# Wumpf/yasph2d

Measured on AMD Instinct MI355X. Metric: particle-steps/sec (whole node), 2D DFSPH dam-break, higher is better.
Workload: dtype f32

## Files before the change

### include/sphx.h

```cpp
#ifndef SPHX_H
#define SPHX_H

#include <stddef.h>
#include <stdint.h>

#ifdef __cplusplus
extern "C" {
#endif

#define SPHX_ABI_VERSION 5

enum {
    SPHX_OK = 0,
    SPHX_ERR_INVALID_ARGUMENT = 1,
    SPHX_ERR_NO_DEVICE = 2,
    SPHX_ERR_HIP = 3,
    SPHX_ERR_NOT_READY = 4,
    SPHX_ERR_NONFINITE = 5,
    SPHX_ERR_NEIGHBOR_PANIC = 6,
    SPHX_ERR_CAPACITY = 7,
    SPHX_ERR_OUT_OF_DOMAIN = 8
};

enum {
// ... 91 lines not shown
typedef struct sphx_render_out {
    uint8_t* rgba;
    uint32_t* owner;
} sphx_render_out;
enum { SPHX_RENDER_NONE = 0xFFFFFFFFu, SPHX_RENDER_BOUNDARY = 0xFFFFFFFEu };
enum { SPHX_RENDER_DEVICE_POINTERS = 1u };
int sphx_render_fit(uint32_t width, uint32_t height, float x, float y, float w, float h, sphx_render_view* out);
int sphx_render(sphx_ctx* ctx, const sphx_render_view* view, uint32_t flags, const sphx_render_out* out);

typedef struct sphx_rect { float x0, y0, x1, y1; } sphx_rect;
#define SPHX_REMOVE_MAX_RECTS 8
enum { SPHX_REMOVE_OUTSIDE = 1u };
int sphx_append(sphx_ctx* ctx, const float* pos_xy, const float* vel_xy , uint32_t m, uint32_t* out_first_id );
int sphx_remove(sphx_ctx* ctx, const sphx_rect* rects, uint32_t n_rects, uint32_t flags, uint32_t* out_removed );

#define SPHX_STATE_SECTIONS 9
enum {
    SPHX_STATE_SEC_POSITIONS = 0, SPHX_STATE_SEC_VELOCITIES = 1, SPHX_STATE_SEC_PARTICLE_ID = 2, SPHX_STATE_SEC_DENSITY = 3, SPHX_STATE_SEC_ALPHA = 4,
    SPHX_STATE_SEC_KAPPA = 5, SPHX_STATE_SEC_STIFFNESS = 6, SPHX_STATE_SEC_ACCEL = 7, SPHX_STATE_SEC_BOUNDARY = 8
};
enum { SPHX_STATE_DEVICE_BUFFER = 1u };
int sphx_state_size(sphx_ctx* ctx, uint64_t* out_bytes);
int sphx_state_save(sphx_ctx* ctx, void* buf, uint64_t capacity, uint32_t flags, uint64_t* out_bytes );
int sphx_state_load(sphx_ctx* ctx, const void* buf, uint64_t bytes, uint32_t flags);
int sphx_state_digest(sphx_ctx* ctx, uint64_t* out );
int sphx_state_save_file(sphx_ctx* ctx, const char* path);
int sphx_state_load_file(sphx_ctx* ctx, const char* path);

#define SPHX_TRACK_MAX_IDS 16384
#define SPHX_TRACK_ABSENT  0xFFFFFFFFu
enum { SPHX_TRACK_DEVICE_POINTERS = 1u };
typedef struct sphx_track_out {
    uint32_t* slot;
    float* pos;
    float* vel;
    float* density;
} sphx_track_out;
typedef struct sphx_track_status { uint32_t m, recording, max_frames, every, frames, dropped, reserved[2]; } sphx_track_status;
int sphx_track_set(sphx_ctx* ctx, const uint32_t* ids , uint32_t m);
int sphx_track_fetch(sphx_ctx* ctx, uint32_t flags, const sphx_track_out* out);
int sphx_track_record(sphx_ctx* ctx, uint32_t max_frames, uint32_t every);
int sphx_track_get_status(const sphx_ctx* ctx, sphx_track_status* out);
int sphx_track_read(sphx_ctx* ctx, uint32_t first_frame, uint32_t n_frames, uint32_t flags, float* out );
int sphx_download_by_id(sphx_ctx* ctx, uint32_t first_id, uint32_t count, uint32_t flags, const sphx_track_out* out, uint32_t* out_present );

typedef struct sphx_fields_out {
    float* vel_grad;
    float* divergence;
    float* vorticity;
    float* color_grad;
} sphx_fields_out;
enum { SPHX_FIELDS_DEVICE_POINTERS = 1u };
int sphx_particle_fields(sphx_ctx* ctx, uint32_t flags, const sphx_fields_out* out);

#define SPHX_STATS_MAX_RECTS 8
enum { SPHX_STATS_DEVICE_POINTERS = 1u };
typedef struct sphx_stats_rec {
    uint64_t count;
    uint64_t nonfinite;
    uint64_t density_count;
    uint32_t density_valid;
    uint32_t reserved;
    double sum_pos[2];
    double sum_vel[2];
    double sum_speed_sq;
    double sum_angular;
    double sum_density;
    double sum_density_sq;
    double max_speed_sq;
    float min_pos[2], max_pos[2];
    float min_density, max_density;
} sphx_stats_rec;
typedef struct sphx_stats_frame { uint64_t step; float dt; uint32_t n; } sphx_stats_frame;
typedef struct sphx_stats_status { uint32_t n_rects, recording, max_frames, every, frames, dropped, reserved[2]; } sphx_stats_status;
int sphx_fluid_stats(sphx_ctx* ctx, const sphx_rect* rects , uint32_t n_rects, uint32_t flags, sphx_stats_rec* out );
int sphx_stats_record(sphx_ctx* ctx, const sphx_rect* rects , uint32_t n_rects, uint32_t max_frames, uint32_t every);
int sphx_stats_get_status(const sphx_ctx* ctx, sphx_stats_status* out);
int sphx_stats_read(sphx_ctx* ctx, uint32_t first_frame, uint32_t n_frames, sphx_stats_rec* out ,
                    sphx_stats_frame* info );

int sphx_debug_correction_counts(sphx_ctx* ctx, uint64_t out[3]);
int sphx_debug_quiet_counts(sphx_ctx* ctx, uint64_t out[2]);
int sphx_debug_takeover_counts(sphx_ctx* ctx, uint64_t out[3]);

int sphx_clear_cached(sphx_ctx* ctx);
int sphx_step_begin(sphx_ctx* ctx, float dt_prev, float* out_vmax);
int sphx_step_finish(sphx_ctx* ctx, float dt, sphx_step_stats* out_stats);

typedef struct sphx_timer_law {
    uint32_t adaptive;
    float cfl_factor;
    float particle_diameter;
    uint32_t reserved;
    uint64_t timestep_min_ns;
    uint64_t timestep_max_ns;
    uint64_t simulation_step_ns;
} sphx_timer_law;
int sphx_step_begin_law(sphx_ctx* ctx, float dt_prev, const sphx_timer_law* law, float* out_vmax);

int sphx_wcsph_step_begin(sphx_ctx* ctx, float dt, float* out_vmax);
int sphx_wcsph_step_finish(sphx_ctx* ctx, float dt, sphx_step_stats* out_stats);

int sphx_update_neighborhood(sphx_ctx* ctx);
int sphx_update_densities(sphx_ctx* ctx, int kernel_kind);
int sphx_compute_alpha(sphx_ctx* ctx);

int sphx_download_solver_state(sphx_ctx* ctx, float* alpha, float* kappa, float* stiffness);
int sphx_download_neighbors(sphx_ctx* ctx, uint16_t* counts, uint32_t* lists, uint64_t* out_total_entries);
int sphx_download_cells(sphx_ctx* ctx, int which, uint32_t* first_particle, uint32_t* cidx, uint32_t* out_count);
uint32_t sphx_last_flags(const sphx_ctx* ctx);
int sphx_grid_info(const sphx_ctx* ctx, int which, uint32_t* out4);
int sphx_get_constants(const sphx_ctx* ctx, float* out6);
int sphx_get_viscosity(const sphx_ctx* ctx, uint32_t* model, float* fluid_viscosity, float* normalizer_laplacian);


int sphx_reserve(sphx_ctx* ctx, uint32_t capacity);
int sphx_tile_configure(sphx_ctx* ctx, int axis, uint32_t cell_lo, uint32_t cell_hi, uint32_t halo_cells, int has_left, int has_right);
#define SPHX_MAX_TILE_PEERS 8
typedef struct sphx_tile_rect { uint32_t x0, x1, y0, y1; } sphx_tile_rect;
int sphx_tile_configure_rect(sphx_ctx* ctx, const sphx_tile_rect* own, uint32_t halo_cells, const sphx_tile_rect* peers, uint32_t n_peers);
int sphx_tile_pack_n(sphx_ctx* ctx, void* const* d_send, uint32_t n_send, uint32_t cap_records);
int sphx_tile_apply_n(sphx_ctx* ctx, const void* const* d_recv, uint32_t n_recv, uint32_t cap_records);
int sphx_tile_advect_pack_n(sphx_ctx* ctx, float dt, void* const* d_send, uint32_t n_send, uint32_t cap_records);
int sphx_tile_upload(sphx_ctx* ctx, const float* pos_xy, const float* vel_xy, const uint32_t* ids, uint32_t n);
#define SPHX_HALO_RECORD_BYTES 32
int sphx_tile_pack(sphx_ctx* ctx, void* d_send_left, void* d_send_right, uint32_t cap_records);
int sphx_tile_apply(sphx_ctx* ctx, const void* d_from_left, const void* d_from_right, uint32_t cap_records);
int sphx_tile_count_kept(sphx_ctx* ctx);
int sphx_sub_regrid(sphx_ctx* ctx, uint32_t* out_n_local);
int sphx_sub_regrid_div(sphx_ctx* ctx, uint32_t* out_n_local);
int sphx_sub_regrid_warm(sphx_ctx* ctx, uint32_t* out_n_local);
int sphx_sub_run_ahead(sphx_ctx* ctx, float dt_prev_of_next_step);
int sphx_tile_carry_warmstart(sphx_ctx* ctx, int kappa, int stiffness);
int sphx_tile_defer_advect(sphx_ctx* ctx, int on);
int sphx_tile_band_packs(const sphx_ctx* ctx, uint32_t* out);
int sphx_tile_send_counts(sphx_ctx* ctx, void* const* d_send, uint32_t n_send, uint32_t cap_records, uint32_t* out_counts);
int sphx_sub_nonpressure(sphx_ctx* ctx, float dt_prev, float* out_vmax_sq);
int sphx_sub_predict(sphx_ctx* ctx, float dt);
int sphx_sub_warmstart(sphx_ctx* ctx, int divergence, float dt);
int sphx_sub_iteration(sphx_ctx* ctx, int divergence, float dt, int first, double* out_err_sum, uint64_t* out_n_owned);
int sphx_sub_advect(sphx_ctx* ctx, float dt);
int sphx_sub_predict_iteration(sphx_ctx* ctx, float dt, double* out_err_sum, uint64_t* out_n_owned);


typedef struct sphx_multi sphx_multi;
enum { SPHX_LAYOUT_AUTO = 0, SPHX_LAYOUT_STRIPS = 1, SPHX_LAYOUT_GRID = 2 };
typedef struct sphx_multi_options {
    uint32_t halo_cells;
    uint32_t fixed_halo;
    uint32_t rebalance_every;
    uint32_t layout;
    uint32_t cap_records;
    uint32_t overlap_exchange;
    uint32_t reserved[2];
} sphx_multi_options;
typedef struct sphx_comm_ops {
    void* user;
    int rank, world;
    int (*exchange)(void* user, const int* peers, int n_peers, void* const* d_send, void* const* d_recv, size_t bytes, void* hip_stream);
    int (*allreduce)(void* user, const double* in, int n, int op, double* out);
    void (*abort)(void* user);
} sphx_comm_ops;
typedef struct sphx_multi_info_t {
    uint32_t world, local_tiles, halo_now, halo_max, peers, n_local, cap_records, grid_layout;
    int32_t axis;
    uint32_t band_packs;
// ... 177 lines not shown
```

### yasph2d_amd/__init__.py

```python
import ctypes as C

import numpy as np

from . import _lib
from ._lib import (FLAG_DENSITY_ITER_CAP, FLAG_DIVERGENCE_ITER_CAP, FLAG_DENSE_CELL, FLAG_NEIGHBOR_CAP, FLAG_STRAY_PARTICLES, FLAG_WARMUP, KERNEL_POLY6,
                   KERNEL_SPIKY, KERNEL_WENDLAND_C2, VISCOSITY_PHYSICAL, VISCOSITY_XSPH, SphxError, SphxKernelTime, SphxParams, SphxStepStats)

__all__ = ["SphxContext", "FluidParticleWorld", "TimeManager", "DFSPHSolver", "DFSPHMultiSolver", "default_params", "duration_from_secs_f32",
           "duration_as_secs_f32", "SphxError", "WCSPHSolver", "VISCOSITY_XSPH", "VISCOSITY_PHYSICAL", "SAMPLE_FIELDS", "gauge_elevation",
           "render_fit", "render_merge", "write_png", "SCENE_RECT", "TRACK_FIELDS", "FIELD_NAMES", "STATS_DTYPE", "STATS_FRAME_DTYPE"]


def _p(a):
    return a.ctypes.data_as(C.c_void_p) if a is not None else None


LISTS_32BIT = 0xFFFFFFFF


_VISCOSITY_MODELS = {"xsph": VISCOSITY_XSPH, "physical": VISCOSITY_PHYSICAL}


def default_params(smoothing_factor=2.0, particle_density=10000.0, fluid_density=100.0, device=0, fixed_iterations=(0, 0), viscosity="xsph",
                   fluid_viscosity=None):
# ... 440 lines not shown
            return out
        out = dict(key=np.zeros((h, w), np.uint32), owner=np.zeros((h, w), np.uint32), rgba=np.zeros((h, w, 4), np.uint8))
        o = _lib.SphxRenderLayer(*[(out[k].ctypes.data or 1) for k in ("key", "owner", "rgba")])
        self._chk(self.L.sphx_tile_render_layer(self.h, C.byref(view), 0, C.byref(o)))
        return out

    def track_record(self, max_frames, every=1):
        self._chk(self.L.sphx_track_record(self.h, max_frames, every))

    def track_frames(self, first=0, count=None):
        st = self.track_status()
        if count is None:
            count = max(st["frames"] - first, 0)
        out = np.zeros((count, st["m"], 4), np.float32)
        self._chk(self.L.sphx_track_read(self.h, first, count, 0, _p(out) if out.size else None))
        return out

    def ids_issued(self):
        first = C.c_uint32()
        rc = self.L.sphx_append(self.h, None, None, 0, C.byref(first))
        if rc == _lib.ERR_NOT_READY:
            return 0
        self._chk(rc)
        return first.value

    def download_by_id(self, first=0, count=None, fields=TRACK_FIELDS):
        if count is None:
            count = max(self.ids_issued() - first, 0)
        outs = _track_outputs(fields, count)
        present = C.c_uint32()
        self._chk(self.L.sphx_download_by_id(self.h, first, count, 0, C.byref(_track_struct(outs)), C.byref(present)))
        outs["present"] = present.value
        return outs

    def download_boundary(self):
        xy = np.zeros((self.nb, 2), np.float32)
        ids = np.zeros(self.nb, np.uint32)
        self._chk(self.L.sphx_download_boundary(self.h, _p(xy), _p(ids)))
        return xy, ids

    def download_solver_state(self):
        n = self.n
        a, k, s = (np.zeros(n, np.float32) for _ in range(3))
        self._chk(self.L.sphx_download_solver_state(self.h, _p(a), _p(k), _p(s)))
        return dict(alpha=a, kappa=k, stiffness=s)

    def download_neighbors(self):
        n = self.n
        counts = np.zeros((n, 2), np.uint16)
        total = C.c_uint64()
        self._chk(self.L.sphx_download_neighbors(self.h, _p(counts), None, C.byref(total)))
        lists = np.zeros(total.value, np.uint32)
        self._chk(self.L.sphx_download_neighbors(self.h, None, _p(lists), C.byref(total)))
        start = np.zeros(n + 1, np.uint64)
        np.cumsum(counts[:, 1].astype(np.uint64), out=start[1:])
        return counts, start, lists

    def download_cells(self, static=False):
        m = C.c_uint32()
        self._chk(self.L.sphx_download_cells(self.h, int(static), None, None, C.byref(m)))
        first = np.zeros(m.value, np.uint32)
        cidx = np.zeros(m.value, np.uint32)
        self._chk(self.L.sphx_download_cells(self.h, int(static), _p(first), _p(cidx), C.byref(m)))
        return first, cidx

    def last_flags(self):
        return self.L.sphx_last_flags(self.h)

    def correction_counts(self):
        out = (C.c_uint64 * 3)()
        self._chk(self.L.sphx_debug_correction_counts(self.h, out))
        return int(out[0]), int(out[1]), int(out[2])

    def quiet_counts(self):
        out = (C.c_uint64 * 2)()
        self._chk(self.L.sphx_debug_quiet_counts(self.h, out))
        return int(out[0]), int(out[1])

    def takeover_counts(self):
        out = (C.c_uint64 * 3)()
        self._chk(self.L.sphx_debug_takeover_counts(self.h, out))
        return int(out[0]), int(out[1]), int(out[2])

    def grid_info(self, which=0):
        out = (C.c_uint32 * 4)()
        self._chk(self.L.sphx_grid_info(self.h, which, out))
        return dict(blocks=out[0], entries=out[1], nbx=out[2], nby=out[3])

    def constants(self):
        out = np.zeros(6, np.float32)
        self._chk(self.L.sphx_get_constants(self.h, _p(out)))
        return out

    def viscosity(self):
        m, mu, nlap = C.c_uint32(), C.c_float(), C.c_float()
        self._chk(self.L.sphx_get_viscosity(self.h, C.byref(m), C.byref(mu), C.byref(nlap)))
        return {VISCOSITY_XSPH: "xsph", VISCOSITY_PHYSICAL: "physical"}[m.value], np.float32(mu.value), np.float32(nlap.value)

    def sample(self, points, kernel=KERNEL_WENDLAND_C2, fields=SAMPLE_FIELDS):
        flags = _sample_fields(fields)
        if _is_torch(points):
            import torch

            if points.device.type != "cuda" or points.dtype != torch.float32 or points.dim() != 2 or points.shape[1] != 2:
                raise ValueError("points must be a float32 [m, 2] tensor on the context's device")
            if self.params is not None and points.device.index not in (None, self.params.device):
                raise ValueError("points are on %s, the context on device %d" % (points.device, self.params.device))
            pts = points.contiguous()
            m = pts.shape[0]
            outs = _torch_outputs(flags, (m,), pts.device)
            torch.cuda.current_stream(pts.device).synchronize()
            self._chk(self.L.sphx_sample_points(self.h, C.c_void_p(pts.data_ptr()), m, kernel, _lib.SAMPLE_DEVICE_POINTERS,
                                                C.byref(_out_struct(outs, lambda t: t.data_ptr()))))
            self.synchronize()
            return outs
        pts = np.ascontiguousarray(points, np.float32)
        if pts.ndim != 2 or pts.shape[1] != 2:
            raise ValueError("points must be a float32 [m, 2] array, not shape %s" % (pts.shape,))
        m = len(pts)
        outs = _numpy_outputs(flags, (m,))
        self._chk(self.L.sphx_sample_points(self.h, _p(pts), m, kernel, 0, C.byref(_out_struct(outs, lambda a: a.ctypes.data))))
        return outs

    def sample_grid(self, origin, spacing, shape, kernel=KERNEL_WENDLAND_C2, fields=SAMPLE_FIELDS):
        flags = _sample_fields(fields)
        dx, dy = (spacing, spacing) if np.ndim(spacing) == 0 else spacing
        ny, nx = (int(v) for v in shape)
        if nx < 0 or ny < 0:
            raise ValueError("shape must be (ny, nx) with non-negative sizes")
        outs = _numpy_outputs(flags, (ny, nx))
        self._chk(self.L.sphx_sample_grid(self.h, origin[0], origin[1], dx, dy, nx, ny, kernel, 0,
                                          C.byref(_out_struct(outs, lambda a: a.ctypes.data))))
        return outs

    def render(self, view=None, *, out=None, owner=False, rgba=True, **view_fields):
        if view is None:
            width, height = view_fields.pop("width", 1920), view_fields.pop("height", 1080)
            view = render_fit(width, height, view_fields.pop("world_rect", SCENE_RECT))
        else:
            view = _copy_view(view)
        _set_view_fields(view, view_fields)
        owner_tensor = owner if _is_torch(owner) else None
        owner = owner_tensor is not None or bool(owner)
        if not rgba and not owner:
            raise ValueError("nothing to render: rgba and owner are both off")
        h, w = view.height, view.width
        o = _lib.SphxRenderOut()
        if out is not None or owner_tensor is not None:
            import torch

            dev = out.device if out is not None else owner_tensor.device
            if out is not None and (not _is_torch(out) or out.device.type != "cuda" or out.dtype != torch.uint8 or tuple(out.shape) != (h, w, 4)
                                    or not out.is_contiguous()):
                raise ValueError("out must be a contiguous uint8 (%d, %d, 4) tensor on the context's device" % (h, w))
            if not rgba and out is not None:
                raise ValueError("out given with rgba=False")
            own = None
            if owner:
                own = owner_tensor if owner_tensor is not None else torch.empty((h, w), dtype=torch.int32, device=dev)
                if own.dtype != torch.int32 or tuple(own.shape) != (h, w) or not own.is_contiguous() or own.device != dev:
                    raise ValueError("owner must be a contiguous int32 (%d, %d) tensor on the device of out" % (h, w))
            o.rgba = (out.data_ptr() or 1) if out is not None else None
            o.owner = (own.data_ptr() or 1) if own is not None else None
            torch.cuda.current_stream(dev).synchronize()
            self._chk(self.L.sphx_render(self.h, C.byref(view), _lib.RENDER_DEVICE_POINTERS, C.byref(o)))
            self.synchronize()
# ... 367 lines not shown
```

### yasph2d_amd/_lib.py

```python
import ctypes as C
import os
import subprocess

_HERE = os.path.dirname(os.path.abspath(__file__))
LIB_PATH = os.environ.get("SPHX_LIB") or os.path.join(_HERE, "libsphx.so")
CSRC = os.path.join(_HERE, "csrc")

OK, ERR_INVALID_ARGUMENT, ERR_NO_DEVICE, ERR_HIP, ERR_NOT_READY, ERR_NONFINITE, ERR_NEIGHBOR_PANIC, ERR_CAPACITY, ERR_OUT_OF_DOMAIN = range(9)
FLAG_NEIGHBOR_CAP, FLAG_DENSITY_ITER_CAP, FLAG_DIVERGENCE_ITER_CAP, FLAG_WARMUP, FLAG_STRAY_PARTICLES, FLAG_DENSE_CELL = 1, 2, 4, 8, 16, 32
KERNEL_WENDLAND_C2, KERNEL_POLY6, KERNEL_SPIKY = 0, 1, 2
VISCOSITY_XSPH, VISCOSITY_PHYSICAL = 0, 1


class SphxParams(C.Structure):
    _fields_ = [
        ("smoothing_length", C.c_float),
        ("particle_mass", C.c_float),
        ("fluid_density", C.c_float),
        ("particle_radius", C.c_float),
        ("gravity", C.c_float * 2),
        ("grid_min", C.c_float * 2),
        ("xsph_epsilon", C.c_float),
        ("max_avg_density_error", C.c_float),
        ("max_density_iterations", C.c_uint32),
# ... 137 lines not shown
    _fields_ = [("fixed", C.c_uint32), ("cfl_factor", C.c_float), ("timestep_max_ns", C.c_uint64), ("timestep_min_ns", C.c_uint64),
                ("simulation_step_ns", C.c_uint64), ("timestep_target_frame_ns", C.c_uint64), ("total_simulated_ns", C.c_uint64),
                ("num_simulation_steps", C.c_uint32), ("reserved", C.c_uint32)]


class SphxMultiOptions(C.Structure):
    _fields_ = [("halo_cells", C.c_uint32), ("fixed_halo", C.c_uint32), ("rebalance_every", C.c_uint32), ("layout", C.c_uint32),
                ("cap_records", C.c_uint32), ("overlap_exchange", C.c_uint32), ("reserved", C.c_uint32 * 2)]


COMM_EXCHANGE = C.CFUNCTYPE(C.c_int, C.c_void_p, C.POINTER(C.c_int), C.c_int, C.POINTER(C.c_void_p), C.POINTER(C.c_void_p), C.c_size_t, C.c_void_p)
COMM_ALLREDUCE = C.CFUNCTYPE(C.c_int, C.c_void_p, C.POINTER(C.c_double), C.c_int, C.c_int, C.POINTER(C.c_double))
COMM_ABORT = C.CFUNCTYPE(None, C.c_void_p)


class SphxCommOps(C.Structure):
    _fields_ = [("user", C.c_void_p), ("rank", C.c_int), ("world", C.c_int), ("exchange", COMM_EXCHANGE), ("allreduce", COMM_ALLREDUCE),
                ("abort", COMM_ABORT)]


class SphxMultiInfo(C.Structure):
    _fields_ = [("world", C.c_uint32), ("local_tiles", C.c_uint32), ("halo_now", C.c_uint32), ("halo_max", C.c_uint32), ("peers", C.c_uint32),
                ("n_local", C.c_uint32), ("cap_records", C.c_uint32), ("grid_layout", C.c_uint32), ("axis", C.c_int32), ("band_packs", C.c_uint32),
                ("exchanges", C.c_uint64), ("rebalances", C.c_uint64), ("build_particles", C.c_uint64), ("neighbor_entries", C.c_uint64),
                ("remote_entries", C.c_uint64), ("owned_local", C.c_uint64), ("transport", C.c_char * 96),
                ("halo_bytes_packed", C.c_uint64), ("halo_bytes_sent", C.c_uint64), ("ownership_seconds", C.c_double)]


LAYOUT_AUTO, LAYOUT_STRIPS, LAYOUT_GRID = 0, 1, 2

_vp, _u16p = C.c_void_p, C.c_void_p
_f, _u32, _u64, _i = C.c_float, C.c_uint32, C.c_uint64, C.c_int
class SphxTileStateOut(C.Structure):
    _fields_ = [(k, C.c_void_p) for k in ("pos", "vel", "id", "density", "alpha", "kappa", "stiffness")]


SIGNATURES = {
    "sphx_abi_version": (_u32, []),
    "sphx_default_params": (_i, [_f, _f, _f, C.POINTER(SphxParams)]),
    "sphx_create": (_i, [C.POINTER(SphxParams), C.POINTER(_vp)]),
    "sphx_destroy": (None, [_vp]),
    "sphx_last_error": (C.c_char_p, [_vp]),
    "sphx_set_boundary": (_i, [_vp, _vp, _u32]),
    "sphx_upload": (_i, [_vp, _vp, _vp, _u32]),
    "sphx_append": (_i, [_vp, _vp, _vp, _u32, C.POINTER(_u32)]),
    "sphx_remove": (_i, [_vp, C.POINTER(SphxRect), _u32, _u32, C.POINTER(_u32)]),
    "sphx_state_size": (_i, [_vp, C.POINTER(_u64)]),
    "sphx_state_save": (_i, [_vp, _vp, _u64, _u32, C.POINTER(_u64)]),
    "sphx_state_load": (_i, [_vp, _vp, _u64, _u32]),
    "sphx_state_digest": (_i, [_vp, C.POINTER(_u64)]),
    "sphx_state_save_file": (_i, [_vp, C.c_char_p]),
    "sphx_state_load_file": (_i, [_vp, C.c_char_p]),
    "sphx_track_set": (_i, [_vp, _vp, _u32]),
    "sphx_track_fetch": (_i, [_vp, _u32, C.POINTER(SphxTrackOut)]),
    "sphx_track_record": (_i, [_vp, _u32, _u32]),
    "sphx_track_get_status": (_i, [_vp, C.POINTER(SphxTrackStatus)]),
    "sphx_track_read": (_i, [_vp, _u32, _u32, _u32, _vp]),
    "sphx_particle_fields": (_i, [_vp, _u32, C.POINTER(SphxFieldsOut)]),
    "sphx_fluid_stats": (_i, [_vp, C.POINTER(SphxRect), _u32, _u32, _vp]),
    "sphx_stats_record": (_i, [_vp, C.POINTER(SphxRect), _u32, _u32, _u32]),
    "sphx_stats_get_status": (_i, [_vp, C.POINTER(SphxStatsStatus)]),
    "sphx_stats_read": (_i, [_vp, _u32, _u32, _vp, _vp]),
    "sphx_tile_fluid_stats": (_i, [_vp, C.POINTER(SphxRect), _u32, _u32, _vp]),
    "sphx_tile_stats_record": (_i, [_vp, C.POINTER(SphxRect), _u32, _u32, _u32]),
    "sphx_tile_stats_frame": (_i, [_vp, _f, _u32]),
    "sphx_tile_stats_read": (_i, [_vp, _u32, _u32, _vp, _vp]),
    "sphx_multi_fluid_stats": (_i, [_vp, C.POINTER(SphxRect), _u32, _u32, _vp, _vp]),
    "sphx_multi_stats_record": (_i, [_vp, C.POINTER(SphxRect), _u32, _u32, _u32]),
    "sphx_multi_stats_get_status": (_i, [_vp, C.POINTER(SphxStatsStatus)]),
    "sphx_multi_stats_read": (_i, [_vp, _u32, _u32, _vp, _vp]),
    "sphx_tile_state_pack": (_i, [_vp, _u32, C.POINTER(SphxTileStateOut), C.POINTER(_u64), C.POINTER(_u32)]),
    "sphx_tile_state_fetch": (_i, [_vp, C.POINTER(_u64), C.POINTER(_u32)]),
    "sphx_tile_upload_state": (_i, [_vp, _vp, _vp, _vp, _vp, _vp, _u32]),
    "sphx_get_tiling_invariant": (_i, [_vp]),
    "sphx_multi_state_size": (_i, [_vp, C.POINTER(_u64)]),
    "sphx_multi_state_save": (_i, [_vp, _vp, _u64, _u32, C.POINTER(_u64)]),
    "sphx_multi_state_load": (_i, [_vp, C.POINTER(_vp), C.POINTER(_u64), _u32, _u32]),
    "sphx_multi_state_digest": (_i, [_vp, C.POINTER(_u64)]),
    "sphx_multi_state_save_file": (_i, [_vp, C.c_char_p]),
    "sphx_multi_state_load_file": (_i, [_vp, C.c_char_p]),
    "sphx_debug_correction_counts": (_i, [_vp, _vp]),
    "sphx_debug_quiet_counts": (_i, [_vp, _vp]),
    "sphx_debug_takeover_counts": (_i, [_vp, _vp]),
    "sphx_download_by_id": (_i, [_vp, _u32, _u32, _u32, C.POINTER(SphxTrackOut), C.POINTER(_u32)]),
    "sphx_download": (_i, [_vp, _vp, _vp, _vp, _vp]),
    "sphx_download_boundary": (_i, [_vp, _vp, _vp]),
    "sphx_num_particles": (_u32, [_vp]),
    "sphx_num_boundary": (_u32, [_vp]),
    "sphx_sample_points": (_i, [_vp, _vp, _u32, _i, _u32, C.POINTER(SphxSampleOut)]),
    "sphx_sample_grid": (_i, [_vp, _f, _f, _f, _f, _u32, _u32, _i, _u32, C.POINTER(SphxSampleOut)]),
    "sphx_render_fit": (_i, [_u32, _u32, _f, _f, _f, _f, C.POINTER(SphxRenderView)]),
    "sphx_render": (_i, [_vp, C.POINTER(SphxRenderView), _u32, C.POINTER(SphxRenderOut)]),
    "sphx_multi_render": (_i, [_vp, C.POINTER(SphxRenderView), _u32, C.POINTER(SphxRenderOut)]),
    "sphx_multi_render_layer": (_i, [_vp, C.POINTER(SphxRenderView), _u32, C.POINTER(SphxRenderLayer)]),
    "sphx_render_merge": (_i, [_u32, _u32, C.POINTER(SphxRenderLayer), _u32, C.POINTER(SphxRenderLayer)]),
    "sphx_tile_render_layer": (_i, [_vp, C.POINTER(SphxRenderView), _u32, C.POINTER(SphxRenderLayer)]),
    "sphx_tile_render_window": (_i, [_vp, C.POINTER(SphxRenderView), _u32, C.POINTER(_u32), C.POINTER(SphxRenderLayer)]),
    "sphx_clear_cached": (_i, [_vp]),
    "sphx_step_begin": (_i, [_vp, _f, C.POINTER(_f)]),
    "sphx_step_begin_law": (_i, [_vp, _f, _vp, _vp]),
    "sphx_timer_law_of": (_i, [_vp, _f, _vp]),
    "sphx_timer_set_target_frame": (None, [_vp, _u64]),
    "sphx_timer_on_step_started": (None, [_vp]),
    "sphx_step_finish": (_i, [_vp, _f, C.POINTER(SphxStepStats)]),
    "sphx_update_neighborhood": (_i, [_vp]),
    "sphx_update_densities": (_i, [_vp, _i]),
    "sphx_compute_alpha": (_i, [_vp]),
    "sphx_download_solver_state": (_i, [_vp, _vp, _vp, _vp]),
    "sphx_download_neighbors": (_i, [_vp, _vp, _vp, C.POINTER(_u64)]),
    "sphx_download_cells": (_i, [_vp, _i, _vp, _vp, C.POINTER(_u32)]),
    "sphx_grid_info": (_i, [_vp, _i, C.POINTER(_u32)]),
    "sphx_last_flags": (_u32, [_vp]),
    "sphx_get_constants": (_i, [_vp, _vp]),
    "sphx_get_viscosity": (_i, [_vp, C.POINTER(_u32), C.POINTER(_f), C.POINTER(_f)]),
    "sphx_reserve": (_i, [_vp, _u32]),
    "sphx_tile_configure": (_i, [_vp, _i, _u32, _u32, _u32, _i, _i]),
    "sphx_tile_upload": (_i, [_vp, _vp, _vp, _vp, _u32]),
    "sphx_tile_pack": (_i, [_vp, _vp, _vp, _u32]),
    "sphx_tile_apply": (_i, [_vp, _vp, _vp, _u32]),
    "sphx_tile_count_kept": (_i, [_vp]),
    "sphx_sub_regrid": (_i, [_vp, C.POINTER(_u32)]),
    "sphx_sub_regrid_div": (_i, [_vp, C.POINTER(_u32)]),
    "sphx_sub_regrid_warm": (_i, [_vp, C.POINTER(_u32)]),
    "sphx_sub_nonpressure": (_i, [_vp, _f, C.POINTER(_f)]),
    "sphx_sub_predict": (_i, [_vp, _f]),
    "sphx_sub_warmstart": (_i, [_vp, _i, _f]),
    "sphx_sub_iteration": (_i, [_vp, _i, _f, _i, C.POINTER(C.c_double), C.POINTER(_u64)]),
    "sphx_sub_predict_iteration": (_i, [_vp, _f, C.POINTER(C.c_double), C.POINTER(_u64)]),
    "sphx_tile_band_packs": (_i, [_vp, C.POINTER(_u32)]),
    "sphx_tile_send_counts": (_i, [_vp, _vp, _u32, _u32, C.POINTER(_u32)]),
    "sphx_sub_advect": (_i, [_vp, _f]),
    "sphx_shm_open": (_vp, [C.c_char_p, _i, _i]),
    "sphx_shm_allreduce": (_i, [_vp, _vp, _i, _i, _vp]),
    "sphx_shm_allgather": (_i, [_vp, _vp, _i, _vp]),
    "sphx_shm_abort": (None, [_vp]),
    "sphx_sub_run_ahead": (_i, [_vp, C.c_float]),
    "sphx_tile_carry_warmstart": (_i, [_vp, _i, _i]),
    "sphx_set_tiling_invariant": (_i, [_vp, _i]),
    "sphx_tile_defer_advect": (_i, [_vp, _i]),
    "sphx_build_stats": (_i, [_vp, _vp, _vp, _vp]),
    "sphx_shm_close": (None, [_vp]),
    "sphx_tile_configure_rect": (_i, [_vp, _vp, _u32, _vp, _u32]),
    "sphx_tile_pack_n": (_i, [_vp, _vp, _u32, _u32]),
    "sphx_tile_apply_n": (_i, [_vp, _vp, _u32, _u32]),
    "sphx_tile_advect_pack_n": (_i, [_vp, _f, _vp, _u32, _u32]),
    "sphx_view_request": (_i, [_vp, _u32, C.POINTER(_u32)]),
    "sphx_view_fetch": (_i, [_vp, _i, C.POINTER(C.POINTER(_f)), C.POINTER(_u32)]),
    "sphx_synchronize": (_i, [_vp]),
    "sphx_set_stream": (_i, [_vp, _vp]),
    "sphx_profile_enable": (_i, [_vp, _i]),
    "sphx_profile_reset": (_i, [_vp]),
    "sphx_profile_filter": (_i, [_vp, C.c_char_p, _u32]),
    "sphx_profile_get": (_i, [_vp, _vp, C.POINTER(_u32)]),
    "sphx_profile_event_overhead": (_i, [_vp, C.POINTER(C.c_double)]),
    "sphx_multi_default_options": (_i, [C.POINTER(SphxMultiOptions)]),
    "sphx_multi_create": (_i, [C.POINTER(SphxParams), C.POINTER(C.c_int), _i, C.POINTER(SphxMultiOptions), C.POINTER(_vp)]),
    "sphx_multi_create_rank": (_i, [C.POINTER(SphxParams), _i, C.POINTER(SphxCommOps), C.c_char_p, _i, _i, C.POINTER(SphxMultiOptions), C.POINTER(_vp)]),
    "sphx_multi_destroy": (None, [_vp]),
    "sphx_multi_last_error": (C.c_char_p, [_vp]),
    "sphx_multi_set_layout": (_i, [_vp, _i, _vp, _u32]),
    "sphx_multi_set_grid_layout": (_i, [_vp, _u32, _u32, _vp, _vp]),
    "sphx_multi_set_boundary": (_i, [_vp, _vp, _u32]),
    "sphx_multi_upload": (_i, [_vp, _vp, _vp, _vp, _u32]),
    "sphx_multi_clear_cached": (_i, [_vp]),
    "sphx_multi_step_begin": (_i, [_vp, _f, C.POINTER(_f)]),
    "sphx_multi_step_finish": (_i, [_vp, _f, C.POINTER(SphxStepStats)]),
# ... 87 lines not shown
```

### yasph2d_amd/csrc/sphx_handoff.hpp

```cpp
#pragma once
#include <cstdint>
#include <cstring>

namespace sphx {

struct BuildHandoff {
    enum Kind : uint8_t { None, WarmApplied, FirstErrors };
    Kind kind = None;
    bool has_flags = false, warm_taken = false;
    uint32_t mark_tag = 0;
    struct Taken {
        bool fused, flags_usable, warm_taken;
    };
    static BuildHandoff warm_applied() { return BuildHandoff{WarmApplied, false, false, 0u}; }
    static BuildHandoff first_errors(bool flags, uint32_t tag, bool taken) { return BuildHandoff{FirstErrors, flags, flags && taken, tag}; }
    void clear() { *this = BuildHandoff{}; }
    bool first_errors_pending() const { return kind == FirstErrors; }
    bool take_warm() {
        const bool applied = kind == WarmApplied;
        if (applied) clear();
        return applied;
    }
    Taken take_first_errors(bool first_divergence, uint32_t rseq) {
        if (kind != FirstErrors || !first_divergence) return Taken{false, false, false};
        const bool usable = has_flags && mark_tag == rseq;
        const Taken t{true, usable, usable && warm_taken};
        clear();
        return t;
    }
};

class PendingCount {
  public:
    enum class Maker : uint8_t { Nobody, Correction, Pack, Classifier };
    PendingCount() = default;
    void made_by_correction(uint32_t n) { *this = PendingCount(Maker::Correction, n); }
    void made_by_pack(uint32_t n) { *this = PendingCount(Maker::Pack, n); }
    void made_by_classifier(uint32_t n, float dt) { *this = PendingCount(Maker::Classifier, n, true, bits(dt)); }
    bool live() const { return maker_ != Maker::Nobody; }
    bool from_classifier() const { return maker_ == Maker::Classifier; }
    bool is_for(uint32_t n) const { return live() && n_ == n; }
    bool is_for_first_of(uint32_t n) const { return live() && n_ <= n; }
    uint32_t n() const { return n_; }
    bool take_over_class(uint32_t n, float dt) {
        const bool mine = from_classifier() && takeable_ && n_ == n && dt_bits_ == bits(dt);
        if (mine) made_by_pack(n);
        return mine;
    }
    void bar_take_over() { takeable_ = false; }
    bool drop() {
        const bool wipe = live();
        forget();
        return wipe;
    }
    bool drop_if_from_classifier() { return from_classifier() && drop(); }
    void forget() { *this = PendingCount(); }

  private:
    PendingCount(Maker m, uint32_t n, bool takeable = false, uint32_t dt_bits = 0) : maker_(m), takeable_(takeable), n_(n), dt_bits_(dt_bits) {}
    static uint32_t bits(float f) {
        uint32_t u;
        std::memcpy(&u, &f, 4);
        return u;
    }
    Maker maker_ = Maker::Nobody;
    bool takeable_ = false;
    uint32_t n_ = 0, dt_bits_ = 0;
};

}
```

### yasph2d_amd/csrc/sphx_internal.hpp

```cpp
#pragma once
#include <hip/hip_runtime.h>

#include <dlfcn.h>

#include <algorithm>
#include <cstdint>
#include <cstdlib>
#include <cstdio>
#include <cstring>
#include <functional>
#include <map>
#include <string>
#include <vector>

#include "../../include/sphx.h"
#include "sphx_handoff.hpp"

namespace sphx {

constexpr uint32_t EMPTY = 0xFFFFFFFFu;
constexpr uint32_t MAX_NEIGHBORS = 64;
constexpr uint32_t BLOCK_SHIFT = 6;
constexpr uint32_t BLOCK_CELLS = 4096;
constexpr uint32_t SCAN_TILE = 4096;
// ... 27 lines not shown
constexpr uint32_t RANK_LOOP_MAX = 4096;
constexpr uint32_t LOOP_HIST = 512;

constexpr uint32_t MAX_TILE_PEERS = 8;
struct TileRect {
    uint32_t x0, x1, y0, y1;
};

struct Consts {
    float h;
    float radius_sq;
    float cell_inv;
    float gmin_x, gmin_y;
    float w_hinv, w_norm, w_ngrad;
    float p6_hsq, p6_norm, p6_ngrad;
    float sp_h, sp_norm, sp_ngrad;
    float mass, rho0, xsph_eps;
    float ax, ay;
    float gx, gy;
    float wc_stiffness, wc_boundary_force;
    TileRect tile;
    uint32_t remote_cap;
    uint32_t q_noclamp;
    uint32_t nt_cold;
    uint32_t xcd_shift;
    uint32_t rev;
};

struct ViscConsts {
    uint32_t visc_model;
    float mu;
    float vis_nlap;
};
template <int VM>
struct ViscArg {};
template <>
struct ViscArg<SPHX_VISCOSITY_PHYSICAL> : ViscConsts {};

struct NbView {
    const uint32_t* list;
    const uint16_t* counts;
    const uint32_t* wave;
    const uint32_t* remote;
    uint32_t lazy_hi;
    uint32_t stream;
};
constexpr uint32_t COUNT_MANY_LINES = 1u << 14;
struct PVr {
    const float2* pos;
    const float2* vel;
};

struct GridView {
    const uint32_t* dir;
    const uint2* fine;
    uint32_t bx0, by0, nbx, nby;
    uint32_t cbits;
};
struct NbGrid {
    const uint32_t* dirn;
    const uint2* fine;
    uint32_t bx0, by0, nbx, nbx1, nby1;
};
constexpr uint32_t DIRN_FLAG = 1u;

struct alignas(128) Stripe {
    unsigned long long nb_entries;
    unsigned long long owned;
    unsigned long long rem_entries;
    unsigned long long res_hi, res_lo;
    uint32_t ticket;
    uint32_t pad0;
    unsigned long long zs_skipped, zs_window, zs_remote;
    unsigned long long zs_quiet;
    uint32_t pad[12];
};
static_assert(sizeof(Stripe) == 128, "one stripe, one cache line");
struct alignas(128) VmaxStripe {
    uint32_t vmax[4];
    uint32_t pad[28];
};
struct alignas(128) MarkStripe {
    uint32_t knz_mark;
    uint32_t pad[31];
};
struct alignas(128) SpecLine {
    uint32_t flags;
    uint32_t pad0;
    unsigned long long moved;
    uint32_t pad[28];
};
struct DevScalars {
    uint32_t flags;
    uint32_t ticket;
    uint32_t sort_total;
    float dt;
    uint32_t loop_done;
    uint32_t pad0;
    unsigned long long snap_hi[2], snap_lo[2];
    uint32_t pad[18];
    Stripe stripe[STRIPES];
    VmaxStripe vstripe[STRIPES];
    MarkStripe mstripe[STRIPES];
    SpecLine spec;
};

struct Mailbox {
    volatile uint32_t seq;
    uint32_t flags;
    uint32_t vmax_sq_bits;
    uint32_t quiet_seq;
    double err_sum;
    unsigned long long nb_entries;
    unsigned long long owned_cum;
    unsigned long long rem_entries;
    uint32_t sort_total;
    uint32_t dt_bits;
    unsigned long long dt_ns;
    volatile uint32_t loop_gen_done;
    uint32_t loop_iters;
    double loop_hist[LOOP_HIST];
    uint32_t send_counts[MAX_TILE_PEERS];
};

struct ResArgs {
    uint32_t enabled;
    uint32_t rseq;
    Mailbox* mb;
    uint32_t seq;
};
struct VmaxArgs {
    uint32_t enabled;
    uint32_t vslot;
    Mailbox* mb;
    uint32_t seq;
};
struct LoopArgs {
    uint32_t enabled;
    uint32_t iter;
    uint32_t fixed;
    uint32_t max_iters;
    uint32_t gen;
    uint32_t n_total;
    float tol;
    float rho0;
    float dt;
};

struct TimerLaw {
    uint32_t enabled, adaptive;
    float cfl_factor, particle_diameter;
    unsigned long long min_ns, max_ns, step_ns;
};

struct Grid {
    uint32_t* dir = nullptr;
    uint32_t* dirn = nullptr;
    uint32_t dir_cap = 0;
    uint2* fine = nullptr;
    uint32_t* hist = nullptr;
    uint32_t* tile_empty = nullptr;
    uint32_t tile_cap = 0;
    uint32_t fine_cap = 0;
    uint32_t bx0 = 0, by0 = 0, nbx = 0, nby = 0, nblk = 0;
    std::vector<uint8_t> cover;
    std::vector<uint32_t> h_dir;
    bool fine_valid = false;
    uint32_t len() const { return nblk * BLOCK_CELLS; }
    uint32_t cbits_floor = 1;
    uint32_t cbits() const {
        uint32_t b = cbits_floor < 1u ? 1u : cbits_floor > 31u ? 31u : cbits_floor;
        while (b < 31u && ((1u << b) - 1u) < len()) ++b;
        return b;
    }
    GridView view() const { return GridView{dir, fine, bx0, by0, nbx, nby, cbits()}; }
    NbGrid nview() const { return nbx && nby ? NbGrid{dirn, fine, bx0, by0, nbx, nbx - 1u, nby - 1u} : NbGrid{dirn, fine, 0u, 0u, 1u, 0u, 0u}; }
};

struct ProfTotals {
    uint64_t launches = 0;
    double ms = 0, bytes = 0;
};
struct ProfPending {
    const char* name;
    double bytes;
    hipEvent_t a, b;
};

}

struct sphx_ctx {
    sphx_params P;
    sphx::Consts K;
    sphx::ViscConsts VK;
    int device = 0;
    hipStream_t stream = nullptr;
    std::string err;

    uint32_t N = 0, capN = 0;
    uint32_t B = 0, capB = 0;
    uint32_t cached_n = 0;
    bool set_changed = false;
    uint64_t ids_issued = 0;
    uint32_t* edit_buf = nullptr;
    uint32_t edit_cap = 0;
    struct Track {
        uint32_t m = 0, unique = 0, log2_bits = 0;
        uint32_t* set_buf = nullptr;
        uint32_t *table = nullptr, *map = nullptr, *filter = nullptr, *found = nullptr;
        float* rec = nullptr;
        uint32_t recording = 0, max_frames = 0, every = 0, frames = 0, dropped = 0, steps = 0;
        uint32_t* scratch = nullptr;
        size_t scratch_cap = 0;
    } track;
    struct Stats {
        sphx_stats_rec* scratch = nullptr;
        sphx_stats_rec* rec = nullptr;
        sphx_rect rects[SPHX_STATS_MAX_RECTS] = {};
        uint32_t n_rects = 0, recording = 0, max_frames = 0, every = 0, frames = 0, dropped = 0, steps = 0;
        std::vector<sphx_stats_frame> info;
    } stats;
    bool uploaded = false, boundary_changed = true, tails_dirty = true, in_step = false;
    bool lists_current = false;
    unsigned long long* state_dig = nullptr;
    uint32_t* mstate_buf = nullptr;
    size_t mstate_cap = 0;
    uint32_t mstate_n = 0;
    uint32_t fast_walk_ok = 0;
    uint32_t sample_ready = 0;
    bool tile_density_ready = false;
    const char* sample_missing = "no neighbour build yet: run a step, or sphx_update_neighborhood + sphx_update_densities";
    float* sample_buf = nullptr;
    size_t sample_cap = 0;
    uint32_t* render_buf = nullptr;
    size_t render_cap = 0;
    float* fields_buf = nullptr;
    size_t fields_cap = 0;
    uint32_t num_density_iters = 1, num_divergence_iters = 0;
    float step_dt_prev = 0, step_vmax = 0;
    uint32_t step_flags = 0;

    float2 *posA = nullptr, *posA2 = nullptr;
    float2 *vel = nullptr, *vel2 = nullptr;
    sphx::PVr pv() const { return sphx::PVr{posA, vel}; }
    float* kbuf = nullptr;
    uint32_t* knz = nullptr;
    int zero_skip = -1;
    bool zero_skip_on() const { return zero_skip < 0 ? N >= 4000000u : zero_skip != 0; }
    int zero_skip_count = 0;
    bool quiet_hint[2] = {false, false};
    unsigned long long qf_launches = 0;
    int quiet_takeover = 1;
    uint32_t thin_grid = 0;
    int quiet_takeover_density = 1;
    bool take_over(bool divergence) const {
        return !tile_mode && (divergence || quiet_takeover_density) && (quiet_takeover == 2 || (quiet_takeover == 1 && quiet_hint[divergence ? 1 : 0]));
    }
    unsigned long long thin_launches = 0, takeover_producers = 0;
    float2* accel = nullptr;
    float *density = nullptr, *alpha = nullptr, *alpha2 = nullptr, *kappa = nullptr, *stiff = nullptr;
    float *kappa2 = nullptr, *stiff2 = nullptr;
    uint32_t *pid = nullptr, *pid2 = nullptr;
    uint32_t *key = nullptr, *slot = nullptr, *order = nullptr;
    uint32_t idx_cap = 0;
    uint32_t soff() const { return capN; }
    float2 *bpos = nullptr, *bpos2 = nullptr;
    uint32_t *bid = nullptr, *bid2 = nullptr;
    sphx::Grid gdyn, gstat;
    bool have_fluid_bbox = false;
    uint32_t fb[4] = {0, 0, 0, 0};
    uint32_t builds_since_cover = 0;
    bool need_expand = false;
    bool need_recover = false;
    uint32_t recover_streak = 0;
    uint32_t recover_cooldown = 0;
    std::vector<float> h_boundary;
    uint32_t* nb_list = nullptr;
    uint16_t* nb_counts = nullptr;
    uint32_t* nb_wave = nullptr;
    uint32_t* nb_remote = nullptr;
    uint32_t pre_seq = 0, pre_warm = 0, law_dt_bits = 0;
    bool law_active = false;
    uint32_t pre_gen = 0;
    uint32_t pre_queued = 0;
    uint32_t loop_gen = 0;
    uint32_t res_seq = 0;
    uint32_t vmax_seq = 0;
    struct RunAhead {
        bool queued = false;
        bool valid = false;
        uint32_t n = 0, dt_bits = 0, vslot = 0;
        uint32_t seq = 0;
    } ahead;
    float tile_pending_dt = 0.0f;
    uint32_t tile_pending_n = 0;
    bool tile_defer_advect = false;
    float sub_ahead_dt = 0.0f;
    bool tile_carry_kappa = true, tile_carry_stiff = true;
    bool tiling_invariant = false;
    int run_ahead = 1;
#ifndef SPHX_DEFAULT_FUSE_PREDICT
#define SPHX_DEFAULT_FUSE_PREDICT 1
#endif
    int fuse_predict = SPHX_DEFAULT_FUSE_PREDICT;
    int tile_fuse_class = 1;
    uint32_t tile_band_packs = 0;
    bool tile_fix_owner = false;
    int fuse_div = 1;
    int xcd_chunk = -1;
    int alternate_sweep = 1;
    int fuse_warm = 1;
    sphx::BuildHandoff handoff;
    int host_loop = 0;
    std::string prof_filter;
    uint32_t prof_every = 1, prof_counter = 0;
    bool external_stream = false;
    hipStream_t view_stream = nullptr;
    hipEvent_t view_packed = nullptr, view_done = nullptr;
    float *view_dev = nullptr, *view_host = nullptr;
    uint32_t view_cap = 0, view_count = 0;
    bool view_pending = false;
    uint32_t wcsph_n = 0;
    bool in_wcsph = false;
    int lazy_table = 1;
    int stream_lists = -1;
    int nt_cold_stores = -1;
    sphx::NbView nbv() const {
        return sphx::NbView{nb_list, nb_counts, nb_wave, nb_remote, (uint32_t)lazy_table, stream_lists < 0 ? (N >= 4000000u ? 1u : 0u) : (uint32_t)stream_lists};
    }
    uint32_t* scan_partials = nullptr;
    uint32_t scan_partials_cap = 0;
    unsigned long long* scan_state = nullptr;
    uint32_t scan_state_cap = 0, scan_epoch = 0;
    sphx::PendingCount pending;
    int no_fused_count = 0;
    int scan_two_pass = 0;
    sphx::DevScalars* d_scal = nullptr;
    sphx::Mailbox* mbox = nullptr;
    sphx::Mailbox* mbox_dev = nullptr;
    uint32_t seq = 0;
    unsigned long long nb_cum = 0, nb_last = 0;
    unsigned long long rem_cum = 0, rem_last = 0;
    unsigned long long owned_cum = 0, owned_last = 0, owned_base = 0;
    bool owned_dirty = false;
    bool tile_mode = false;
    uint32_t tile_halo = 0;
    uint32_t tile_npeers = 0;
    sphx::TileRect tile_peer[sphx::MAX_TILE_PEERS] = {};
    uint32_t n_owned = 0;
    uint32_t* tile_blk = nullptr;
    bool tile_strip_left = false, tile_strip_right = false;

    bool profiling = false;
    std::vector<hipEvent_t> ev_pool;
    std::vector<sphx::ProfPending> prof_pending;
    std::map<std::string, sphx::ProfTotals> prof_totals;

    int fail(int code, const char* what, const char* detail = nullptr) {
        quiet_hint[0] = quiet_hint[1] = false;
        err = what;
        if (detail) {
            err += ": ";
            err += detail;
        }
        return code;
    }
};
```

### yasph2d_amd/csrc/sphx_kernels.hip

```cpp
#include "sphx_internal.hpp"
#include "sphx_sqrt.hpp"
#include "sphx_xcd.hpp"

namespace sphx {

__device__ __forceinline__ uint32_t part1by1(uint32_t x) {
    x &= 0xffffu;
    x = (x ^ (x << 8)) & 0x00ff00ffu;
    x = (x ^ (x << 4)) & 0x0f0f0f0fu;
    x = (x ^ (x << 2)) & 0x33333333u;
    x = (x ^ (x << 1)) & 0x55555555u;
    return x;
}
__device__ __forceinline__ uint32_t morton2(uint32_t x, uint32_t y) { return (part1by1(y) << 1) | part1by1(x); }

__device__ __forceinline__ uint32_t spread6(uint32_t v) {
    v &= 63u;
    v = (v | (v << 4)) & 0x30Fu;
    v = (v | (v << 2)) & 0x333u;
    v = (v | (v << 1)) & 0x555u;
    return v;
}
__device__ __forceinline__ uint32_t sat_u16(float v) {
    v = fminf(fmaxf(v, 0.0f), 65535.0f);
// ... 558 lines not shown
    }
    count_cell(K, g, i < n, i, p, hist, cidx, slot, ring, scal);
}

constexpr uint32_t ORDER_HEAD = 0x80000000u, ORDER_INDEX = 0x7FFFFFFFu;
#ifndef SPHX_SCATTER_PER_LANE
#define SPHX_SCATTER_PER_LANE 4
#endif
constexpr uint32_t SCATTER_PER_LANE = SPHX_SCATTER_PER_LANE;
__global__ __launch_bounds__(256) void k_scatter(const uint32_t* __restrict__ cidx, const uint32_t* __restrict__ slot, uint32_t n,
                                                  const uint2* __restrict__ fine, uint32_t* __restrict__ order, uint32_t cbits,
                                                  uint32_t* __restrict__ hist, uint32_t rev) {
    const uint32_t b0 = xcd_bid(xcd_packed_rev(rev), xcd_packed_shift(rev)) * (256u * SCATTER_PER_LANE) + threadIdx.x;
    if (b0 - threadIdx.x >= n) return;
    uint32_t w[SCATTER_PER_LANE];
#pragma unroll
    for (uint32_t u = 0; u < SCATTER_PER_LANE; ++u) w[u] = b0 + u * 256u < n ? cidx[b0 + u * 256u] : EMPTY;
    uint32_t first[SCATTER_PER_LANE];
#pragma unroll
    for (uint32_t u = 0; u < SCATTER_PER_LANE; ++u) first[u] = fine[w[u] == EMPTY ? 0u : w[u] & ((1u << cbits) - 1u)].x;
#ifdef SPHX_SLOT_AT_COUNT
    (void)hist;
#pragma unroll
    for (uint32_t u = 0; u < SCATTER_PER_LANE; ++u) {
        if (w[u] == EMPTY) continue;
        const uint32_t i = b0 + u * 256u;
        uint32_t sl = w[u] >> cbits;
        if (sl == cell_slot_max(cbits)) sl = slot[i];
        const uint32_t p = first[u] + sl;
        if (p < n) order[p] = i | (sl == 0u ? ORDER_HEAD : 0u);
    }
#else
    (void)slot;
    const uint32_t lane = threadIdx.x & 63u;
    uint32_t old[SCATTER_PER_LANE], pos_in_run[SCATTER_PER_LANE];
#pragma unroll
    for (uint32_t u = 0; u < SCATTER_PER_LANE; ++u) {
        const uint32_t idx = w[u];
        const uint32_t prev = dpp_mov<0x138>(idx, idx);
        const bool head = (lane == 0) || (idx != prev);
        const unsigned long long mask = __ballot(head);
        const uint32_t start = 63u - (uint32_t)__clzll(mask & (~0ull >> (63u - lane)));
        const unsigned long long rest = (lane == 63) ? 0ull : (mask >> (lane + 1));
        const uint32_t end = rest ? lane + (uint32_t)__ffsll((long long)rest) : 64u;
        uint32_t o = 0;
        if (head && idx != EMPTY) o = atomicSub(&hist[idx], end - lane);
        old[u] = o;
        pos_in_run[u] = (start << 8) | (lane - start);
    }
#pragma unroll
    for (uint32_t u = 0; u < SCATTER_PER_LANE; ++u) {
        const uint32_t o = (uint32_t)__shfl((int)old[u], (int)(pos_in_run[u] >> 8), 64);
        if (w[u] == EMPTY) continue;
        const uint32_t i = b0 + u * 256u;
        const uint32_t sl = o - 1u - (pos_in_run[u] & 0xFFu);
        const uint32_t p = first[u] + sl;
        if (p < n) order[p] = i | (sl == 0u ? ORDER_HEAD : 0u);
    }
#endif
}

struct GatherArgs {
    const float2* pos_in;
    float2* pos_out;
    const float2* vel_in;
    float2* vel_out;
    const float* r_in;
    float* r_out;
    const float* r2_in;
    float* r2_out;
    const float* r3_in;
    float* r3_out;
    const uint32_t* u_in;
    uint32_t* u_out;
    DevScalars* count_owned;
    DevScalars* flags;
    float advect_dt;
    uint32_t advect_below;
    uint32_t fix_owner;
    float cell_inv, gmin_x, gmin_y;
    TileRect own;
    uint32_t rank_by_id;
    uint32_t nt_cold;
};
#ifndef SPHX_GATHER_PER_LANE
#define SPHX_GATHER_PER_LANE 1
#endif
constexpr uint32_t GATHER_PER_LANE = SPHX_GATHER_PER_LANE;
__global__ __launch_bounds__(256) void k_rank_gather(const uint32_t* __restrict__ order, const uint32_t* __restrict__ cidx, uint32_t n,
                                                      uint32_t n_in, const uint2* __restrict__ fine, GatherArgs a,
                                                      const uint32_t* __restrict__ n_dev, uint32_t cbits, uint32_t rev) {
    if (n_dev) n = min(n, *n_dev);
    const uint32_t b0 = xcd_bid(xcd_packed_rev(rev), xcd_packed_shift(rev)) * (256u * GATHER_PER_LANE);
    if (b0 >= n) return;
    constexpr int RANK_L = 5, RANK_R = 6;
    constexpr uint32_t ORD_HALO = 8, SPAN = 256u * GATHER_PER_LANE;
    static_assert(RANK_L <= (int)ORD_HALO && RANK_R <= (int)ORD_HALO, "window of order[] words in LDS");
    __shared__ uint32_t sord[SPAN + 2 * ORD_HALO];
    uint32_t own[GATHER_PER_LANE];
#pragma unroll
    for (uint32_t u = 0; u < GATHER_PER_LANE; ++u) {
        own[u] = order[min(b0 + u * 256u + threadIdx.x, n - 1u)];
        sord[ORD_HALO + u * 256u + threadIdx.x] = own[u];
    }
    if (threadIdx.x < 2 * ORD_HALO) {
        const int32_t k = threadIdx.x < ORD_HALO ? (int32_t)(b0 + threadIdx.x) - (int32_t)ORD_HALO : (int32_t)(b0 + SPAN + threadIdx.x - ORD_HALO);
        sord[threadIdx.x < ORD_HALO ? threadIdx.x : SPAN + threadIdx.x] = order[(uint32_t)min(max(k, 0), (int32_t)n - 1)];
    }
    bool ok[GATHER_PER_LANE];
    float2 q[GATHER_PER_LANE], v[GATHER_PER_LANE];
    float r1[GATHER_PER_LANE], r2[GATHER_PER_LANE], r3[GATHER_PER_LANE];
    uint32_t id[GATHER_PER_LANE];
#pragma unroll
    for (uint32_t u = 0; u < GATHER_PER_LANE; ++u) {
        const uint32_t i = own[u] & ORDER_INDEX;
        ok[u] = b0 + u * 256u + threadIdx.x < n && i < n_in;
        const uint32_t ic = ok[u] ? i : 0u;
        q[u] = a.pos_in[ic];
        v[u] = a.vel_in ? a.vel_in[ic] : make_float2(0.0f, 0.0f);
        r1[u] = a.r_in ? a.r_in[ic] : 0.0f, r2[u] = a.r2_in ? a.r2_in[ic] : 0.0f, r3[u] = a.r3_in ? a.r3_in[ic] : 0.0f;
        id[u] = a.u_in ? a.u_in[ic] : 0u;
    }
    __syncthreads();
#pragma unroll
    for (uint32_t u = 0; u < GATHER_PER_LANE; ++u) {
        if (!ok[u]) continue;
        const uint32_t p = b0 + u * 256u + threadIdx.x, i = own[u] & ORDER_INDEX;
        uint32_t near[RANK_L + RANK_R + 1];
#pragma unroll
        for (int d = -RANK_L; d <= RANK_R; ++d) near[d + RANK_L] = sord[(int)(ORD_HALO + u * 256u + threadIdx.x) + d];
        uint32_t heads_l = 0, heads_r = 0;
#pragma unroll
        for (int d = 0; d <= RANK_L; ++d) heads_l |= (near[RANK_L - d] >> 31) << d;
#pragma unroll
        for (int d = 1; d <= RANK_R; ++d) heads_r |= ((near[RANK_L + d] >> 31) | (p + (uint32_t)d >= n ? 1u : 0u)) << (d - 1);
        uint32_t dst;
        if (heads_l != 0u && heads_r != 0u && !(a.rank_by_id && a.u_in)) {
            const uint32_t below = (uint32_t)__builtin_ctz(heads_l), above = (uint32_t)__builtin_ctz(heads_r) + 1u;
            uint32_t rank = 0;
#pragma unroll
            for (int d = -RANK_L; d <= RANK_R; ++d) {
                if (d == 0) continue;
                const bool mate = d < 0 ? (uint32_t)(-d) <= below : (uint32_t)d < above;
                rank += (mate && (near[d + RANK_L] & ORDER_INDEX) < i) ? 1u : 0u;
            }
            dst = p - below + rank;
        } else {
            const uint32_t cw = cidx[i];
            if (cw == EMPTY) continue;
            const uint2 se = fine[cw & ((1u << cbits) - 1u)];
            const uint32_t s = se.x;
            uint32_t e = se.y;
            if (e > n) e = n;
            if (e - s <= RANK_LOOP_MAX && a.rank_by_id && a.u_in) {
                const uint32_t me = id[u] & 0x7FFFFFFFu;
                uint32_t rank = 0;
                for (uint32_t k = s; k < e; ++k) {
                    const uint32_t j = order[k] & ORDER_INDEX;
                    const uint32_t idj = j < n_in ? a.u_in[j] & 0x7FFFFFFFu : 0xFFFFFFFFu;
                    rank += (j != i && (idj < me || (idj == me && j < i))) ? 1u : 0u;
                }
                dst = s + rank;
            } else if (e - s <= RANK_LOOP_MAX) {
                uint32_t rank = 0;
#pragma unroll
                for (int d = -RANK_L; d <= RANK_R; ++d) {
                    const int32_t k = (int32_t)p + d;
                    rank += (k >= (int32_t)s && k < (int32_t)e && (near[d + RANK_L] & ORDER_INDEX) < i) ? 1u : 0u;
                }
                for (uint32_t k = s; k + RANK_L < p && k < e; ++k) rank += ((order[k] & ORDER_INDEX) < i) ? 1u : 0u;
                for (uint32_t k = max(s, p + RANK_R + 1u); k < e; ++k) rank += ((order[k] & ORDER_INDEX) < i) ? 1u : 0u;
                dst = s + rank;
            } else {
                dst = p;
                if ((__hip_atomic_load(&a.flags->flags, __ATOMIC_RELAXED, __HIP_MEMORY_SCOPE_AGENT) & DF_DENSE_CELL) == 0u) atomicOr(&a.flags->flags, DF_DENSE_CELL);
            }
        }
        if (dst >= n) continue;
        float2 qd = q[u];
        if (a.vel_in) {
            if (a.advect_dt > 0.0f && i < a.advect_below) {
                qd.x = qd.x + v[u].x * a.advect_dt;
                qd.y = qd.y + v[u].y * a.advect_dt;
            }
            a.vel_out[dst] = v[u];
        }
        a.pos_out[dst] = qd;
        if (a.r_in) a.r_out[dst] = r1[u];
        if (a.r2_in) a.r2_out[dst] = r2[u];
        if (a.r3_in) a.r3_out[dst] = r3[u];
        if (a.u_in) {
            uint32_t idd = id[u];
            if (a.fix_owner && i < a.advect_below) {
                const uint32_t cx = sat_u16((qd.x - a.gmin_x) * a.cell_inv), cy = sat_u16((qd.y - a.gmin_y) * a.cell_inv);
                if (!rect_has(a.own, cx, cy, 0u)) idd &= 0x7FFFFFFFu;
            }
            store_cold(&a.u_out[dst], idd, a.nt_cold);
            if (a.count_owned) {
                const unsigned long long m = __ballot((idd >> 31) != 0);
                if (m && (threadIdx.x & 63) == (uint32_t)(__ffsll((long long)__ballot(1)) - 1))
                    atomicAdd(&a.count_owned->stripe[blockIdx.x % STRIPES].owned, (unsigned long long)__popcll(m));
            }
        }
    }
}

__global__ __launch_bounds__(256) void k_iota(uint32_t* __restrict__ a, uint32_t n) {
    const uint32_t i = blockIdx.x * 256 + threadIdx.x;
    if (i < n) a[i] = i;
}
__global__ __launch_bounds__(256) void k_fill_f32(float* __restrict__ a, uint32_t from, uint32_t n, float v) {
    const uint32_t i = from + blockIdx.x * 256 + threadIdx.x;
    if (i < n) a[i] = v;
}
__global__ __launch_bounds__(256) void k_advect(float2* __restrict__ posA, const float2* __restrict__ vel, uint32_t n, float dt) {
    const uint32_t i = xcd_bid() * 256 + threadIdx.x;
    if (i >= n) return;
    float2 p = posA[i];
    const float2 v = vel[i];
    p.x = p.x + v.x * dt;
    p.y = p.y + v.y * dt;
    posA[i] = p;
}
struct HaloRec {
    float4 pv;
    uint32_t id;
    float kappa, stiff;
    uint32_t pad;
};
struct TilePeers {
    uint32_t n;
    TileRect rect[MAX_TILE_PEERS];
    HaloRec* out[MAX_TILE_PEERS];
};
__device__ __forceinline__ uint32_t tile_send_mask(const Consts& K, const TileRect* rect, uint32_t nrect, uint32_t halo, float4 pv, uint32_t id) {
    const bool owned = (id >> 31) != 0 && pv.x == pv.x;
    if (!owned) return 0u;
    uint32_t cx, cy;
    cell_of(K, make_float2(pv.x, pv.y), cx, cy);
    uint32_t m = 0;
    for (uint32_t k = 0; k < nrect; ++k) m |= rect_has(rect[k], cx, cy, halo) ? (1u << k) : 0u;
    return m;
}
__device__ __forceinline__ uint32_t tile_send_mask(const Consts& K, const TilePeers& P, uint32_t halo, float4 pv, uint32_t id) {
    return tile_send_mask(K, P.rect, P.n, halo, pv, id);
}
struct TileClassArgs {
    const uint32_t* pid;
    uint32_t* blk;
    uint32_t* any;
    uint32_t halo, n;
    TileRect rect[MAX_TILE_PEERS];
};
__device__ __forceinline__ float4 tile_advected(float4 pv, float dt) {
    if (dt > 0.0f) {
        pv.x = pv.x + pv.z * dt;
        pv.y = pv.y + pv.w * dt;
    }
    return pv;
}
__global__ __launch_bounds__(256) void k_tile_count(PVr PV, const uint32_t* __restrict__ pid, uint32_t n, Consts K,
                                                     uint32_t halo, TilePeers P, uint32_t* __restrict__ blk, float dt) {
    __shared__ uint32_t wc[4][MAX_TILE_PEERS];
    const uint32_t i = blockIdx.x * 256 + threadIdx.x;
    const uint32_t m = i < n ? tile_send_mask(K, P, halo, tile_advected(ldpv(PV, i), dt), pid[i]) : 0u;
    for (uint32_t k = 0; k < P.n; ++k) {
        const uint32_t c = (uint32_t)__popcll(__ballot((m >> k) & 1u));
        if ((threadIdx.x & 63) == 0) wc[threadIdx.x >> 6][k] = c;
    }
    __syncthreads();
    if (threadIdx.x < P.n) blk[(size_t)blockIdx.x * MAX_TILE_PEERS + threadIdx.x] = wc[0][threadIdx.x] + wc[1][threadIdx.x] + wc[2][threadIdx.x] + wc[3][threadIdx.x];
}
__global__ __launch_bounds__(1024) void k_tile_offsets(uint32_t* __restrict__ blk, uint32_t nb, TilePeers P) {
    __shared__ uint32_t part[1024];
    const uint32_t per = (nb + 1023u) / 1024u;
    const uint32_t b0 = threadIdx.x * per, b1 = min(b0 + per, nb);
    for (uint32_t k = 0; k < P.n; ++k) {
        uint32_t acc = 0;
        for (uint32_t b = b0; b < b1; ++b) acc += blk[(size_t)b * MAX_TILE_PEERS + k];
        part[threadIdx.x] = acc;
        __syncthreads();
        for (uint32_t off = 1; off < 1024; off <<= 1) {
            const uint32_t v = threadIdx.x >= off ? part[threadIdx.x - off] : 0u;
            __syncthreads();
            part[threadIdx.x] += v;
            __syncthreads();
// ... 1125 lines not shown
}
__device__ __forceinline__ uint32_t wave_vmax_get(const DevScalars* __restrict__ scal, uint32_t vslot) {
    const uint32_t lane = threadIdx.x & 63u;
    const uint32_t b = lane < STRIPES ? scal->vstripe[lane].vmax[vslot & 3u] : 0u;
    return wave_max_u32(b);
}
__device__ __forceinline__ void vmax_publish(DevScalars* __restrict__ scal, const VmaxArgs& va, uint32_t bits, const TimerLaw& law, unsigned long long ns,
                                             float dt_new) {
    if (threadIdx.x < STRIPES) __hip_atomic_store(&scal->vstripe[threadIdx.x].vmax[(va.vslot + 2u) & 3u], 0u, __ATOMIC_RELAXED, __HIP_MEMORY_SCOPE_AGENT);
    if (threadIdx.x == 0) {
        va.mb->vmax_sq_bits = bits;
        if (law.enabled) {
            __hip_atomic_store((uint32_t*)&scal->dt, __float_as_uint(dt_new), __ATOMIC_RELAXED, __HIP_MEMORY_SCOPE_AGENT);
            va.mb->dt_ns = ns;
            va.mb->dt_bits = __float_as_uint(dt_new);
        }
    }
    publish_common(scal, va.mb, va.seq);
}

__device__ __forceinline__ unsigned long long residual_fixed(float e, bool& bad) {
    bad = !(e < 1073741824.0f);
    const float t = __builtin_rintf((bad ? 0.0f : e) * 16777216.0f);
    const uint32_t bits = __float_as_uint(t);
    const uint32_t m = (bits & 0x7fffffu) | 0x800000u;
    const int sh = (int)((bits >> 23) & 0xffu) - 150;
    unsigned long long f = sh >= 0 ? (unsigned long long)m << (sh & 63) : (unsigned long long)(m >> min(-sh, 31));
    return (bits & 0x7f800000u) ? f : 0ull;
}
__device__ __forceinline__ void block_residual_add(float e, DevScalars* __restrict__ scal) {
    bool bad;
    const unsigned long long f = wave_sum_u63(residual_fixed(e, bad));
    __shared__ unsigned long long ws[4];
    if ((threadIdx.x & 63) == 0) ws[threadIdx.x >> 6] = f;
    if (__any(bad) && (threadIdx.x & 63) == 0) atomicOr(&scal->flags, DF_NONFINITE);
    __syncthreads();
    if (threadIdx.x == 0) {
        const unsigned long long t = ws[0] + ws[1] + ws[2] + ws[3];
        Stripe* st = &scal->stripe[blockIdx.x % STRIPES];
        if (t >> 32) atomicAdd(&st->res_hi, t >> 32);
        if (t & 0xffffffffull) atomicAdd(&st->res_lo, t & 0xffffffffull);
    }
}
__device__ __forceinline__ void residual_stripe_load(const DevScalars* __restrict__ scal, unsigned long long& hi, unsigned long long& lo) {
    const uint32_t lane = threadIdx.x & 63u;
    hi = lane < STRIPES ? scal->stripe[lane].res_hi : 0ull;
    lo = lane < STRIPES ? scal->stripe[lane].res_lo : 0ull;
}
__device__ __forceinline__ void residual_wave_reduce(unsigned long long& hi, unsigned long long& lo) {
    hi = wave_sum_u63(hi);
    lo = wave_sum_u63(lo);
}
__device__ __forceinline__ double residual_sum_f64(unsigned long long hi, unsigned long long lo, unsigned long long hi0, unsigned long long lo0) {
    return ((double)(hi - hi0) * 4294967296.0 + (double)(lo - lo0)) * (1.0 / 16777216.0);
}

__global__ __launch_bounds__(256) void k_block_occupancy(const uint2* __restrict__ fine, uint32_t nblk, uint8_t* __restrict__ occ) {
    const uint32_t b = blockIdx.x * 256 + threadIdx.x;
    if (b >= nblk) return;
    occ[b] = fine[(size_t)b * BLOCK_CELLS].x != fine[(size_t)b * BLOCK_CELLS + BLOCK_CELLS - 1].y ? 1 : 0;
}

__global__ __launch_bounds__(64) void k_clear_vmax_slot(DevScalars* scal, uint32_t vslot) {
    if (threadIdx.x < STRIPES) __hip_atomic_store(&scal->vstripe[threadIdx.x].vmax[vslot & 3u], 0u, __ATOMIC_RELAXED, __HIP_MEMORY_SCOPE_AGENT);
}

__global__ __launch_bounds__(64) void k_publish_vmax(DevScalars* scal, VmaxArgs va) {
    const uint32_t b = wave_vmax_get(scal, va.vslot);
    vmax_publish(scal, va, b, TimerLaw{}, 0ull, 0.0f);
}

#ifndef NONP_BOUNDS
#define NONP_BOUNDS __launch_bounds__(256) __attribute__((amdgpu_waves_per_eu(8, 8)))
#endif
__device__ __forceinline__ float physical_visc(const Consts& K, const ViscConsts& V, float mu_m, float r, float rho_j) {
    return mu_m * (V.vis_nlap * (K.h - r)) / rho_j;
}
template <int VM>
__global__ NONP_BOUNDS void k_nonpressure(PVr PV, const float* __restrict__ density, uint32_t n, uint32_t soff, Consts K,
                                                      float dt, NbView nb, float2* __restrict__ accel, DevScalars* __restrict__ scal, uint32_t vslot,
                                                      ViscArg<VM> V) {
    __shared__ Stage<2, 1> rec;
    const uint32_t blk = xcd_bid(K.rev, K.xcd_shift);
    const uint32_t i = blk * 256 + threadIdx.x;
    NbHead h = nb_head(nb, blk, i, n);
    struct StageRec {
        float4 pv;
        float rho;
    };
    nb_stage(
        h, nb, blk, i, n, [&](uint32_t g) { return StageRec{ldpv(PV, g), gat(density, g < soff ? g : 0u)}; },
        [&](uint32_t g) {
            const Pair<float4> pv = ldpv2(PV, g);
            const Pair<float> rho = gat2(density, g < soff ? g : 0u);
            return Pair<StageRec>{StageRec{pv.a, rho.a}, StageRec{pv.b, rho.b}};
        },
        [&](uint32_t slot, const StageRec& r) {
            rec.put_vec01(slot, r.pv);
            rec.put_scal<0>(slot, r.rho);
        });
    __syncthreads();
    float vsq = 0.0f;
    if (i < n) {
        const uint32_t oi = (i - h.lw0) * 4u;
        const float4 pvi = h.wide ? ldpv(PV, i) : rec.vec01(oi);
        const uint32_t cd = h.cd;
        float ax = K.ax, ay = K.ay;
        struct Rec {
            float4 pv;
            float rho;
        };
        if constexpr (VM == SPHX_VISCOSITY_PHYSICAL) {
            const float mu_m = V.mu * K.mass;
            auto walk = [&](auto fast) {
                auto consume = [&](const Rec& r, uint32_t) {
                    const float dx = r.pv.x - pvi.x, dy = r.pv.y - pvi.y;
                    const float r_sq = dx * dx + dy * dy;
                    const float f = physical_visc(K, V, mu_m, sqrt_dist<decltype(fast)::value>(r_sq), r.rho);
                    ax = ax + f * (r.pv.z - pvi.z);
                    ay = ay + f * (r.pv.w - pvi.w);
                };
                nb_traverse(
                    h, cd, [&](uint32_t o) { return Rec{rec.vec01(o), rec.scal<0>(o)}; },
                    [&](uint32_t g) { return Rec{ldpv(PV, g), gat(density, g)}; }, consume);
            };
            if (K.q_noclamp)
                walk(std::true_type{});
            else
                walk(std::false_type{});
        } else {
            const float em = K.xsph_eps * K.mass;
            auto consume = [&](const Rec& r, uint32_t) {
                const float dx = r.pv.x - pvi.x, dy = r.pv.y - pvi.y;
                const float r_sq = dx * dx + dy * dy;
                const float f = em * poly6_eval(K, r_sq) / (r.rho * dt);
                ax = ax + f * (r.pv.z - pvi.z);
                ay = ay + f * (r.pv.w - pvi.w);
            };
            nb_traverse(
                h, cd, [&](uint32_t o) { return Rec{rec.vec01(o), rec.scal<0>(o)}; },
                [&](uint32_t g) { return Rec{ldpv(PV, g), gat(density, g)}; }, consume);
        }
        accel[i] = make_float2(ax, ay);
        const float px = pvi.z + ax * dt, py = pvi.w + ay * dt;
        vsq = tile_owns(K, pvi.x, pvi.y) ? px * px + py * py : 0.0f;
    }
    block_vmax_add(vsq, scal, vslot, (uint32_t*)&rec.raw[0]);
}

__global__ __launch_bounds__(256) void k_predict(float2* __restrict__ vel, const float2* __restrict__ accel, uint32_t n, float dt,
                                                  DevScalars* __restrict__ scal, VmaxArgs va, TimerLaw law) {
    const uint32_t i = xcd_bid() * 256 + threadIdx.x;
    const uint32_t il = min(i, n - 1u);
    float2 v = vel[il];
    const float2 a = accel[il];
    if (va.enabled) {
        __shared__ float dt_s;
        if (threadIdx.x < 64) {
            const uint32_t b = wave_vmax_get(scal, va.vslot);
            unsigned long long ns = 0;
            float d = dt;
            if (law.enabled) {
                ns = timer_law_step_ns(law, sqrtf(__uint_as_float(b)));
                d = duration_as_secs_f32(ns);
            }
            if (threadIdx.x == 0) dt_s = d;
            if (blockIdx.x == 0) vmax_publish(scal, va, b, law, ns, d);
        }
        __syncthreads();
        dt = dt_s;
    }
    if (i >= n) return;
    v.x = v.x + a.x * dt;
    v.y = v.y + a.y * dt;
    vel[i] = v;
}

__global__ __launch_bounds__(256) void k_wcsph_leapfrog1(float2* __restrict__ vel, float2* __restrict__ posA, const float2* __restrict__ accel,
                                                          uint32_t n, float dt) {
    const uint32_t i = xcd_bid() * 256 + threadIdx.x;
    if (i >= n) return;
    const float2 p0 = posA[i], v0 = vel[i];
    float4 pv = make_float4(p0.x, p0.y, v0.x, v0.y);
    const float2 a = accel[i];
    const float hdt = 0.5f * dt;
    pv.z = pv.z + hdt * a.x;
    pv.w = pv.w + hdt * a.y;
    pv.x = pv.x + pv.z * dt;
    pv.y = pv.y + pv.w * dt;
    vel[i] = make_float2(pv.z, pv.w);
    posA[i] = make_float2(pv.x, pv.y);
}
__device__ __forceinline__ float powi7(float a) {
    float r = a;
    a = a * a;
    r = r * a;
    a = a * a;
    return r * a;
}
__device__ __forceinline__ float wcsph_pressure(const Consts& K, float local_density) {
    return K.wc_stiffness * (powi7(fmaxf(local_density / K.rho0, 1.0f)) - 1.0f);
}
template <int VM>
__global__ TRAV_BOUNDS void k_wcsph_accel(PVr PV, const float* __restrict__ density, uint32_t n, uint32_t soff, Consts K,
                                          float dt, NbView nb, float2* __restrict__ accel, DevScalars* __restrict__ scal, uint32_t vslot,
                                          ViscArg<VM> V) {
    __shared__ Stage<2, 1> rec;
    const uint32_t blk = xcd_bid(K.rev, K.xcd_shift);
    const uint32_t i = blk * 256 + threadIdx.x;
    NbHead h = nb_head(nb, blk, i, n);
    struct StageRec {
        float4 pv;
        float rho;
    };
    nb_stage(
        h, nb, blk, i, n, [&](uint32_t g) { return StageRec{ldpv(PV, g), gat(density, g < soff ? g : 0u)}; },
        [&](uint32_t g) {
            const Pair<float4> pv = ldpv2(PV, g);
            const Pair<float> rho = gat2(density, g < soff ? g : 0u);
            return Pair<StageRec>{StageRec{pv.a, rho.a}, StageRec{pv.b, rho.b}};
        },
        [&](uint32_t slot, const StageRec& r) {
            rec.put_vec01(slot, r.pv);
            rec.put_scal<0>(slot, r.rho);
        });
    __syncthreads();
    float vsq = 0.0f;
    if (i < n) {
        const uint32_t oi = (i - h.lw0) * 4u;
        const float4 pvi = h.wide ? ldpv(PV, i) : rec.vec01(oi);
// ... 288 lines not shown
```

### yasph2d_amd/csrc/sphx_launch.inc

```
#include <algorithm>
#include <cmath>

using namespace sphx;

static std::string g_create_error;

#define SPHX_HIP(ctx, expr)                                                        \
    do {                                                                           \
        hipError_t e__ = (expr);                                                   \
        if (e__ != hipSuccess) return (ctx)->fail(SPHX_ERR_HIP, #expr, hipGetErrorString(e__)); \
    } while (0)

namespace {

inline uint32_t nblocks(uint32_t n, uint32_t per = 256) {
    const uint32_t b = (n + per - 1) / per;
    return per == 256 ? (b + 7u) & ~7u : b;
}
inline double kbar_of(const sphx_ctx* c) { return (c->N && c->nb_last) ? (double)c->nb_last / (double)c->N : 12.0; }
inline double list_bytes(const sphx_ctx* c) {
    if (!c->K.remote_cap) return 2.0 + 4.0 * kbar_of(c);
    const double rbar = c->N ? (double)c->rem_last / (double)c->N : 0.5;
    return 2.0 + 4.0 / 64.0 + (4.0 / 3.0) * kbar_of(c) + 4.0 * rbar + 4.0 / 256.0;
}
// ... 413 lines not shown
    if (!got) {
        SPHX_HIP(c, hipStreamSynchronize(c->stream));
        if (!reached()) return c->fail(SPHX_ERR_HIP, "device did not publish the step scalars (kernel fault?)");
    }
    __atomic_thread_fence(__ATOMIC_ACQUIRE);
    const unsigned long long cum = c->mbox->nb_entries;
    if (cum != c->nb_cum) {
        c->nb_last = cum - c->nb_cum;
        c->nb_cum = cum;
    }
    const unsigned long long rm = c->mbox->rem_entries;
    if (rm != c->rem_cum) {
        c->rem_last = rm - c->rem_cum;
        c->rem_cum = rm;
    }
    const unsigned long long ow = c->mbox->owned_cum;
    if (ow != c->owned_cum) {
        c->owned_last = ow - c->owned_cum;
        c->owned_cum = ow;
    }
    const uint32_t f = c->mbox->flags;
    if (f) hipLaunchKernelGGL(k_clear_flags, dim3(1), dim3(1), 0, c->stream, c->d_scal, f);
    if (f & DF_NB_CAP) c->step_flags |= SPHX_FLAG_NEIGHBOR_CAP;
    if (f & DF_HALO_CAP) return c->fail(SPHX_ERR_CAPACITY, "halo exchange buffer too small for the particles near a tile cut");
    if (f & DF_NEAR_EDGE) c->need_expand = true;
    if (f & DF_STRAY) {
        c->step_flags |= SPHX_FLAG_STRAY_PARTICLES;
        c->need_recover = true;
    }
    if (f & DF_DENSE_CELL) c->step_flags |= SPHX_FLAG_DENSE_CELL;
    if (f & DF_SCAN_STALL) return c->fail(SPHX_ERR_HIP, "the cell-table scan stalled waiting for a predecessor workgroup");
    if (f & DF_NONFINITE) return c->fail(SPHX_ERR_NONFINITE, "a solver residual is not finite (dfsph.rs:223 / :378 assert)");
    if (f & DF_OUT_OF_DOMAIN) return c->fail(SPHX_ERR_OUT_OF_DOMAIN, "a particle left the Morton domain the grid tables were sized for, or has no cell at all (a NaN position)");
    if (f & DF_NB_PANIC) return c->fail(SPHX_ERR_NEIGHBOR_PANIC, "64 dynamic neighbours and a static hit (neighborhood_search.rs:373 panics here)");
    return SPHX_OK;
}

int publish_and_wait(sphx_ctx* c) {
    const uint32_t seq = ++c->seq;
    hipLaunchKernelGGL(k_publish, dim3(1), dim3(64), 0, c->stream, c->d_scal, c->mbox_dev, seq);
    return wait_mailbox(c, seq);
}

void wipe_histogram(sphx_ctx* c, Grid& g) {
    if (g.hist && g.len()) hipMemsetAsync(g.hist, 0, (size_t)g.len() * 4, c->stream);
}
void drop_fused_count(sphx_ctx* c) {
    if (c->pending.drop()) wipe_histogram(c, c->gdyn);
}
void clear_histograms(sphx_ctx* c) {
    c->pending.forget();
    for (Grid* g : {&c->gdyn, &c->gstat}) wipe_histogram(c, *g);
}

void drop_class_count(sphx_ctx* c) {
    if (c->pending.drop_if_from_classifier()) wipe_histogram(c, c->gdyn);
}
void flush_pending_advect(sphx_ctx* c) {
    if (c->pending.from_classifier() || c->tile_pending_dt > 0.0f) (void)hipSetDevice(c->device);
    drop_class_count(c);
    if (!(c->tile_pending_dt > 0.0f)) return;
    const uint32_t n = c->tile_pending_n;
    const float dt = c->tile_pending_dt;
    c->tile_pending_dt = 0.0f;
    c->tile_pending_n = 0;
    const bool fix = c->tile_fix_owner;
    c->tile_fix_owner = false;
    if (!n) return;
    if (fix) {
        TilePeers none{};
        hipLaunchKernelGGL(k_tile_pack, dim3(nblocks(n)), dim3(256), 0, c->stream, (const float2*)c->vel, c->posA, c->pid, (const float*)c->kappa,
                           (const float*)c->stiff, n, c->K, c->tile_halo, none, (const uint32_t*)c->tile_blk, 0u, dt, CountArgs{}, c->d_scal, 1u,
                           (const uint32_t*)nullptr);
        return;
    }
    hipLaunchKernelGGL(k_advect, dim3(nblocks(n)), dim3(256), 0, c->stream, c->posA, (const float2*)c->vel, n, dt);
}

void sub_step_enter(sphx_ctx* c) {
    c->ahead.valid = false;
    flush_pending_advect(c);
}

int build_grid(sphx_ctx* c, Grid& g, const float2* pos, uint32_t n, const GatherArgs& ga, float advect_dt, bool ring, uint32_t* tile_n = nullptr) {
    hipStream_t st = c->stream;
    DevScalars* ds = c->d_scal;
    const uint32_t len = g.len();
    const uint32_t nt = nblocks(len, c->scan_two_pass ? SCAN_TILE : SCAN1_TILE);
    const bool counted = &g == &c->gdyn && advect_dt > 0 && !tile_n && c->pending.is_for(n);
    const bool partial = &g == &c->gdyn && tile_n && advect_dt == 0.0f && !counted && c->pending.is_for_first_of(n);
    const uint32_t first = partial ? c->pending.n() : 0u;
    if (counted || partial)
        c->pending.forget();
    else
        drop_fused_count(c);
    if (n > first && !counted) {
        const uint32_t gbc = std::max(1u, nblocks(n - first));
        if (advect_dt > 0)
            launch(c, "advect+cell_count", (16.0 + 4 + 4) * n, [&] {
                hipLaunchKernelGGL(k_key_count<true>, dim3(gbc), dim3(256), 0, st, c->pv(), (const float2*)nullptr, n, advect_dt, c->K,
                                   g.view(), g.hist, c->key, c->slot, ring ? 1u : 0u, ds, first);
            });
        else
            launch(c, "cell_count", (8.0 + 4 + 4) * (n - first), [&] {
                hipLaunchKernelGGL(k_key_count<false>, dim3(gbc), dim3(256), 0, st, PVr{nullptr, nullptr}, pos, n, 0.0f, c->K, g.view(),
                                   g.hist, c->key, c->slot, ring ? 1u : 0u, ds, first);
            });
    }
    if (!len) hipMemsetAsync(&ds->sort_total, 0, 4, st);
    uint32_t scan_seq = 0;
    if (len)
        launch(c, "cell_scan", (c->scan_two_pass ? 20.0 : 16.0) * len, [&] {
            if (c->scan_two_pass) {
                hipLaunchKernelGGL(k_scan_reduce, dim3(nt), dim3(256), 0, st, (const uint32_t*)g.hist, len, c->scan_partials, ds, &ds->sort_total);
                hipLaunchKernelGGL(k_scan_apply, dim3(nt), dim3(256), 0, st, g.hist, g.fine, len, (const uint32_t*)c->scan_partials);
                hipMemsetAsync(g.tile_empty, 0, (size_t)g.tile_cap * 4, st);
            } else {
                if (++c->scan_epoch == 0) c->scan_epoch = 1;
                if (tile_n) scan_seq = ++c->seq;
                hipLaunchKernelGGL(k_scan_onepass, dim3(nt), dim3(256), 0, st, g.hist, g.fine, len, c->scan_state, c->scan_epoch, ds, &ds->sort_total,
                                   tile_n ? c->mbox_dev : (Mailbox*)nullptr, scan_seq, g.tile_empty, tile_n ? 0xFFFFFFFFu : n);
            }
        });
    g.fine_valid = len != 0;
    if (n) {
        launch(c, "cell_scatter", 12.0 * n, [&] {
            hipLaunchKernelGGL(k_scatter, dim3((nblocks(n, 256 * SCATTER_PER_LANE) + 7u) & ~7u), dim3(256), 0, st, (const uint32_t*)c->key, (const uint32_t*)c->slot, n, (const uint2*)g.fine,
                               c->order, g.cbits(), g.hist, xcd_scatter_pack(c->K.rev, xcd_shift_of(c)));
        });
        const uint32_t ng = n;
        if (tile_n) {
            if (scan_seq) {
                *tile_n = scan_seq;
            } else {
                const uint32_t seq = ++c->seq;
                hipLaunchKernelGGL(k_publish, dim3(1), dim3(64), 0, st, ds, c->mbox_dev, seq);
                *tile_n = seq;
            }
        }
        const uint32_t gb2 = std::max(8u, (nblocks(ng, 256 * GATHER_PER_LANE) + 7u) & ~7u);
        double gbytes = 4;
        gbytes += ga.vel_in ? (16 + 16) : 16;
        if (ga.r_in) gbytes += 8;
        if (ga.r2_in) gbytes += 8;
        if (ga.r3_in) gbytes += 8;
        if (ga.u_in) gbytes += 8;
        if (ng)
            launch(c, "gather_attributes", gbytes * ng, [&] {
                hipLaunchKernelGGL(k_rank_gather, dim3(gb2), dim3(256), 0, st, (const uint32_t*)c->order, (const uint32_t*)c->key, ng, n,
                                   (const uint2*)g.fine, ga, tile_n ? (const uint32_t*)&ds->sort_total : (const uint32_t*)nullptr, g.cbits(), xcd_pack(c->K.rev, xcd_shift_of(c)));
            });
    }
    return SPHX_OK;
}

int ensure_index_scratch(sphx_ctx* c) {
    const uint32_t need = std::max(std::max(std::max(c->N, c->capN), c->B), 1u);
    if (need <= c->idx_cap) return SPHX_OK;
    int rc;
    if ((rc = dev_alloc(c, &c->key, need))) return rc;
#ifdef SPHX_SLOT_AT_COUNT
    if ((rc = dev_alloc(c, &c->slot, need))) return rc;
#endif
    if ((rc = dev_alloc(c, &c->order, need))) return rc;
    SPHX_HIP(c, hipMemsetAsync(c->order, 0, (size_t)need * 4, c->stream));
    c->idx_cap = need;
    return SPHX_OK;
}

static inline void sample_went_stale(sphx_ctx* c, const char* missing) {
    c->sample_ready = 0u;
    c->tile_density_ready = false;
    c->sample_missing = missing;
}
static inline void sample_after_step(sphx_ctx* c) {
    if (c->sample_ready == 1u)
        c->sample_ready = 2u;
    else
        sample_went_stale(c, "no neighbour build has run since the particles or the boundary changed (a step over zero fluid particles runs "
                             "none): call sphx_update_neighborhood + sphx_update_densities");
}
void track_take_frame(sphx_ctx* c);
static inline void track_after_step(sphx_ctx* c) {
    if (c->track.recording) track_take_frame(c);
}
void stats_take_frame(sphx_ctx* c, float dt);
static inline void stats_after_step(sphx_ctx* c, float dt) {
    if (c->stats.recording) stats_take_frame(c, dt);
}
static inline void lists_went_stale(sphx_ctx* c) {
    c->K.q_noclamp = 0u;
    c->lists_current = false;
    c->quiet_hint[0] = c->quiet_hint[1] = false;
    if (c->d_scal) hipMemsetAsync(&c->d_scal->spec.flags, 0, sizeof(uint32_t), c->stream);
    if (c->sample_ready) sample_went_stale(c, "the positions changed since the last neighbour build: run a step, or sphx_update_neighborhood + sphx_update_densities");
}

int ensure_nb_arrays(sphx_ctx* c, uint32_t needN, uint32_t needB, bool keep_fluid) {
    const uint32_t newN = std::max(c->capN, needN), newB = std::max(c->capB, std::max(needB, 1u));
    if (newN == c->capN && newB == c->capB && c->vel) return SPHX_OK;
    const size_t tot = (size_t)newN + newB;
    if (tot >= ((size_t)1 << 28)) return c->fail(SPHX_ERR_CAPACITY, "more than 2^28 fluid + boundary slots in one context: split the domain into tiles");
    float2* old_pos = c->posA;
    float2* old_vel = c->vel;
    c->posA = nullptr;
    c->vel = nullptr;
    int rc;
    if ((rc = dev_alloc(c, &c->posA, tot + 4)) || (rc = dev_alloc(c, &c->posA2, tot + 4)) || (rc = dev_alloc(c, &c->vel, tot)) ||
        (rc = dev_alloc(c, &c->vel2, tot)))
        return rc;
    if (keep_fluid && c->N && old_vel) {
        SPHX_HIP(c, hipMemcpyAsync(c->posA, old_pos, (size_t)c->N * 8, hipMemcpyDeviceToDevice, c->stream));
        SPHX_HIP(c, hipMemcpyAsync(c->vel, old_vel, (size_t)c->N * 8, hipMemcpyDeviceToDevice, c->stream));
        SPHX_HIP(c, hipStreamSynchronize(c->stream));
    }
    if (keep_fluid && old_vel && newN == c->capN && c->B && !c->tails_dirty) {
        const size_t off = (size_t)c->capN, nb = std::min<size_t>(c->B, c->capB);
        SPHX_HIP(c, hipMemsetAsync(c->posA + off, 0, ((size_t)newB + 4) * 8, c->stream));
        SPHX_HIP(c, hipMemsetAsync(c->vel + off, 0, (size_t)newB * 8, c->stream));
        SPHX_HIP(c, hipMemcpyAsync(c->posA + off, old_pos + off, nb * 8, hipMemcpyDeviceToDevice, c->stream));
        SPHX_HIP(c, hipMemsetAsync(c->posA2 + off, 0, ((size_t)newB + 4) * 8, c->stream));
        SPHX_HIP(c, hipMemsetAsync(c->vel2 + off, 0, (size_t)newB * 8, c->stream));
        SPHX_HIP(c, hipMemcpyAsync(c->posA2 + off, old_pos + off, nb * 8, hipMemcpyDeviceToDevice, c->stream));
        SPHX_HIP(c, hipStreamSynchronize(c->stream));
    }
    dev_free(&old_pos);
    dev_free(&old_vel);
    c->tails_dirty = true;
    lists_went_stale(c);
    return SPHX_OK;
}

int build_static(sphx_ctx* c) {
    int rc;
    if ((rc = cover_static(c))) return rc;
    GatherArgs ga{};
    ga.flags = c->d_scal;
    ga.pos_in = c->bpos;
    ga.pos_out = c->bpos2;
    ga.u_in = c->bid;
    ga.u_out = c->bid2;
    if ((rc = build_grid(c, c->gstat, c->bpos, c->B, ga, 0.0f, false))) return rc;
    std::swap(c->bpos, c->bpos2);
    std::swap(c->bid, c->bid2);
    c->boundary_changed = false;
    c->tails_dirty = true;
    return SPHX_OK;
}

int fill_tails(sphx_ctx* c) {
    if (c->B)
        hipLaunchKernelGGL(k_fill_tails, dim3(nblocks(c->B)), dim3(256), 0, c->stream, (const float2*)c->bpos, c->B, c->soff(), c->posA, c->posA2,
                           c->vel, c->vel2);
    c->tails_dirty = false;
    return SPHX_OK;
}

int recover_directory(sphx_ctx* c, float advect_dt, uint32_t advect_below = 0xFFFFFFFFu) {
    const uint32_t n = c->N;
    if (!n) return SPHX_OK;
    std::vector<float> hp((size_t)n * 2), hv((size_t)n * 2);
    SPHX_HIP(c, hipMemcpyAsync(hp.data(), c->posA, (size_t)n * 8, hipMemcpyDeviceToHost, c->stream));
    SPHX_HIP(c, hipMemcpyAsync(hv.data(), c->vel, (size_t)n * 8, hipMemcpyDeviceToHost, c->stream));
    SPHX_HIP(c, hipStreamSynchronize(c->stream));
    std::vector<float> xy((size_t)n * 2);
    size_t m = 0;
    for (uint32_t i = 0; i < n; ++i) {
        const float dt_i = i < advect_below ? advect_dt : 0.0f;
        const float x = hp[2 * (size_t)i] + hv[2 * (size_t)i] * dt_i, y = hp[2 * (size_t)i + 1] + hv[2 * (size_t)i + 1] * dt_i;
        if (std::isfinite(x) && std::isfinite(y)) {
            xy[2 * m] = x;
            xy[2 * m + 1] = y;
            m += 1;
        }
    }
    if (!m) return SPHX_OK;
// ... 12 lines not shown
    }
    return cover_dynamic(c, xy.data(), (uint32_t)m, false);
}

inline uint32_t* zero_skip_flags(const sphx_ctx* c) { return c->zero_skip_on() && !c->tile_mode ? c->knz : nullptr; }

int update_neighborhood(sphx_ctx* c, bool extra_alpha, float advect_dt, bool fuse, bool fuse_div = false, bool fuse_warm = false) {
    int rc;
    drop_class_count(c);
    c->lists_current = false;
    sample_went_stale(c, "the last neighbour build did not complete: upload the state again");
    if (c->boundary_changed) {
        if ((rc = build_static(c))) return rc;
    }
    if (c->tails_dirty) fill_tails(c);
    if (c->need_expand) {
        c->need_expand = false;
        if ((rc = cover_dynamic(c, nullptr, 0, true))) return rc;
    } else if (++c->builds_since_cover >= COVER_PERIOD) {
        if ((rc = cover_from_occupancy(c))) return rc;
    }
    const float cover_dt = advect_dt > 0.0f ? advect_dt : (c->tile_pending_dt > 0.0f ? c->tile_pending_dt : 0.0f);
    const uint32_t cover_below = advect_dt > 0.0f ? 0xFFFFFFFFu : c->tile_pending_n;
    if (c->tile_mode && c->gdyn.nblk == 0 && c->N) {
        if ((rc = recover_directory(c, cover_dt, cover_below))) return rc;
    }
    if (c->need_recover) {
        c->need_recover = false;
        c->recover_streak = 8;
    }
    if (c->recover_streak) {
        c->recover_streak -= 1;
        if (c->recover_cooldown) {
            c->recover_cooldown -= 1;
        } else if ((rc = recover_directory(c, cover_dt, cover_below))) {
            return rc;
        }
    }
    GatherArgs ga{};
    ga.flags = c->d_scal;
    ga.pos_in = c->posA;
    ga.pos_out = c->posA2;
    ga.vel_in = c->vel;
    ga.vel_out = c->vel2;
    ga.advect_dt = advect_dt;
    ga.advect_below = 0xFFFFFFFFu;
    if (extra_alpha) {
        ga.r_in = c->alpha;
        ga.r_out = c->alpha2;
    }
    ga.u_in = c->pid;
    ga.u_out = c->pid2;
    uint32_t tile_n = c->N;
    const bool carry_kappa = c->tile_mode ? c->tile_carry_kappa : c->tiling_invariant, carry_stiff = c->tile_mode ? c->tile_carry_stiff : c->tiling_invariant;
    ga.rank_by_id = c->tiling_invariant ? 1u : 0u;
    ga.nt_cold = c->nt_cold_stores < 0 ? (c->N >= NT_COLD_FROM ? 1u : 0u) : (uint32_t)c->nt_cold_stores;
    if (carry_kappa) {
        ga.r2_in = c->kappa;
        ga.r2_out = c->kappa2;
    }
    if (carry_stiff) {
        ga.r3_in = c->stiff;
        ga.r3_out = c->stiff2;
    }
    if (c->tile_mode) ga.count_owned = c->d_scal;
    if (c->tile_pending_dt > 0.0f) {
        if (c->tile_mode && advect_dt == 0.0f && c->pending.is_for(c->tile_pending_n) && c->tile_pending_n <= c->N) {
            ga.advect_dt = c->tile_pending_dt;
            ga.advect_below = c->tile_pending_n;
            c->tile_pending_dt = 0.0f;
            c->tile_pending_n = 0;
            if (c->tile_fix_owner) {
                c->tile_fix_owner = false;
                ga.fix_owner = 1u;
                ga.cell_inv = c->K.cell_inv;
                ga.gmin_x = c->K.gmin_x;
                ga.gmin_y = c->K.gmin_y;
                ga.own = c->K.tile;
            }
        } else {
            flush_pending_advect(c);
        }
    }
    if ((rc = build_grid(c, c->gdyn, c->posA, c->N, ga, advect_dt, true, c->tile_mode ? &tile_n : nullptr))) return rc;
    if (carry_kappa) std::swap(c->kappa, c->kappa2);
    if (carry_stiff) std::swap(c->stiff, c->stiff2);
    std::swap(c->vel, c->vel2);
    std::swap(c->posA, c->posA2);
    if (extra_alpha) std::swap(c->alpha, c->alpha2);
    std::swap(c->pid, c->pid2);
    c->K.q_noclamp = c->fast_walk_ok;
    hipStream_t st = c->stream;
    const uint32_t* n_dev = c->tile_mode ? (const uint32_t*)&c->d_scal->sort_total : (const uint32_t*)nullptr;
    if (c->N) {
        const uint32_t n = c->N;
        auto go = [&](auto kernel, const DivArgs& dv) {
            hipLaunchKernelGGL(kernel, dim3(nblocks(n)), dim3(256), 0, st, (const float2*)c->posA, n, c->soff(), c->K, c->gdyn.nview(), c->gstat.nview(),
                               c->nb_list, c->nb_counts, c->nb_wave, c->nb_remote, c->density, c->alpha, c->d_scal, n_dev, dv);
        };
        c->handoff.clear();
        if (fuse && fuse_warm) {
            DivArgs dv{};
            dv.velw = c->vel;
            dv.warm = c->stiff;
            dv.lim = -0.5f * c->K.rho0 * c->K.rho0;
            launch(c, "neighbor_build+density_alpha+divergence_warmstart", (8.0 + list_bytes(c) + 8.0 + 8.0 + 8.0 + 4.0) * n, [&] { go(k_neighbor_build<3>, dv); });
            c->handoff = BuildHandoff::warm_applied();
        } else if (fuse && fuse_div) {
            DivArgs dv{};
            dv.vel = (const float2*)c->vel;
            dv.kbuf = c->kbuf;
            dv.knz = zero_skip_flags(c);
            dv.knz_tag = c->res_seq + 1u;
            const bool take = dv.knz && c->take_over(true);
            if (take) {
                dv.warm = c->stiff;
                c->takeover_producers += 1;
            }
            launch(c, "neighbor_build+density_alpha+density_change", (8.0 + list_bytes(c) + 8.0 + 8.0 + 4.0) * n,
                   [&] { take ? go(k_neighbor_build<2, true>, dv) : go(k_neighbor_build<2>, dv); });
            c->handoff = BuildHandoff::first_errors(dv.knz != nullptr, dv.knz_tag, take);
        } else if (fuse)
            launch(c, "neighbor_build+density_alpha", (8.0 + list_bytes(c) + 8.0) * n, [&] { go(k_neighbor_build<1>, DivArgs{}); });
        else
            launch(c, "neighbor_build", (8.0 + list_bytes(c)) * n, [&] { go(k_neighbor_build<0>, DivArgs{}); });
    }
    if (c->tile_mode && c->N) {
        if ((rc = wait_mailbox(c, tile_n))) return rc;
        c->N = std::min(c->mbox->sort_total, c->N);
    }
    c->lists_current = true;
    c->sample_ready = 1u;
    c->sample_missing = "the densities of the last neighbour build are missing: call sphx_update_densities";
    return SPHX_OK;
}

template <int KIND>
void launch_density(sphx_ctx* c, bool density, bool alpha) {
    const uint32_t n = c->N;
    if (!n) return;
    const double bytes = (8.0 + list_bytes(c) + (density ? 4 : 0) + (alpha ? 4 : 0)) * n;
    auto go = [&](auto kernel) {
        hipLaunchKernelGGL(kernel, dim3(nblocks(n)), dim3(256), 0, c->stream, (const float2*)c->posA, n, c->soff(), c->K, c->nbv(), c->density, c->alpha);
    };
    if (density && alpha) return launch(c, "density_alpha", bytes, [&] { go(k_density_alpha<KIND, true, true>); });
    if (density) return launch(c, "update_densities", bytes, [&] { go(k_density_alpha<KIND, true, false>); });
    launch(c, "compute_alpha_factors", bytes, [&] { go(k_density_alpha<0, false, true>); });
}

int alloc_particles(sphx_ctx* c, uint32_t n, uint32_t cap = 0, bool keep_set = false) {
    if (n <= c->capN) return SPHX_OK;
    cap = std::max(cap, n);
    int rc = 0;
    if ((rc = ensure_nb_arrays(c, cap, c->capB, keep_set))) return rc;
    float *old_kappa = c->kappa, *old_stiff = c->stiff, *old_alpha = c->alpha;
    float2* old_accel = c->accel;
    uint32_t* old_pid = keep_set ? c->pid : nullptr;
    if (keep_set) c->pid = nullptr;
    const uint32_t keep = std::min(c->cached_n, c->capN);
    const uint32_t keep_accel = std::min(c->wcsph_n, c->capN);
    c->kappa = c->stiff = c->alpha = nullptr;
    c->accel = nullptr;
    auto give_up = [&](int code) {
        dev_free(&old_kappa);
        dev_free(&old_stiff);
        dev_free(&old_alpha);
        dev_free(&old_accel);
        dev_free(&old_pid);
        c->cached_n = 0;
        c->wcsph_n = 0;
        c->uploaded = false;
        return code;
    };
#define A(p) \
    if ((rc = dev_alloc(c, &c->p, cap))) return give_up(rc);
    A(accel) A(density) A(alpha) A(alpha2) A(kappa) A(stiff) A(kappa2) A(stiff2) A(pid) A(pid2) A(nb_counts) A(kbuf)
#undef A
    if ((rc = dev_alloc(c, &c->knz, (size_t)(nblocks(cap) + 8) * 4))) return give_up(rc);
    if ((rc = dev_alloc(c, &c->nb_remote, (size_t)(nblocks(cap) + 8) * REMOTE_CAP))) return give_up(rc);
    if ((rc = dev_alloc(c, &c->nb_wave, (size_t)(nblocks(cap) + 8) * 4))) return give_up(rc);
    const size_t slices = ((size_t)cap + 63) / 64;
    if ((rc = dev_alloc(c, &c->nb_list, slices * 64 * 64))) return give_up(rc);
    SPHX_HIP(c, hipMemsetAsync(c->kappa, 0, (size_t)cap * 4, c->stream));
    SPHX_HIP(c, hipMemsetAsync(c->stiff, 0, (size_t)cap * 4, c->stream));
    SPHX_HIP(c, hipMemsetAsync(c->alpha, 0, (size_t)cap * 4, c->stream));
    SPHX_HIP(c, hipMemsetAsync(c->density, 0, (size_t)cap * 4, c->stream));
    if (keep) {
        SPHX_HIP(c, hipMemcpyAsync(c->kappa, old_kappa, (size_t)keep * 4, hipMemcpyDeviceToDevice, c->stream));
        SPHX_HIP(c, hipMemcpyAsync(c->stiff, old_stiff, (size_t)keep * 4, hipMemcpyDeviceToDevice, c->stream));
        SPHX_HIP(c, hipMemcpyAsync(c->alpha, old_alpha, (size_t)keep * 4, hipMemcpyDeviceToDevice, c->stream));
    }
    if (keep_accel) SPHX_HIP(c, hipMemcpyAsync(c->accel, old_accel, (size_t)keep_accel * 8, hipMemcpyDeviceToDevice, c->stream));
    if (old_pid && c->N) SPHX_HIP(c, hipMemcpyAsync(c->pid, old_pid, (size_t)c->N * 4, hipMemcpyDeviceToDevice, c->stream));
    SPHX_HIP(c, hipStreamSynchronize(c->stream));
    dev_free(&old_kappa);
    dev_free(&old_stiff);
    dev_free(&old_alpha);
    dev_free(&old_accel);
    dev_free(&old_pid);
    c->capN = cap;
    return SPHX_OK;
}

inline bool device_loop(const sphx_ctx* c) { return !c->tile_mode && !c->host_loop; }


void launch_predict(sphx_ctx* c, const char* label, float dt, const VmaxArgs& va = VmaxArgs{}, const TimerLaw& tl = TimerLaw{}) {
    const uint32_t n = c->N;
    launch(c, label, 24.0 * n, [&] { hipLaunchKernelGGL(k_predict, dim3(nblocks(n)), dim3(256), 0, c->stream, c->vel, (const float2*)c->accel, n, dt, c->d_scal, va, tl); });
}

void launch_compute_error(sphx_ctx* c, bool divergence, float dt, const float* dt_dev, const LoopArgs& la, uint32_t* clear_hist, uint32_t clear_len,
                          const PredArgs* pred, uint32_t* knz, uint32_t knz_tag, bool take_warm = false,
                          const CountArgs& take_count = CountArgs{}) {
    const uint32_t n = c->N;
    const double lb = list_bytes(c);
    auto go = [&](auto kernel, float* warm, const PredArgs& pa, auto take) {
        hipLaunchKernelGGL(kernel, dim3(nblocks(n)), dim3(256), 0, c->stream, c->pv(), (const float*)c->density, (const float*)c->alpha, n, c->soff(), c->K, dt,
                           c->nbv(), c->kbuf, warm, c->d_scal, dt_dev, la, clear_hist, clear_len, pa, knz, knz_tag, take);
    };
    if (divergence) {
        launch(c, "compute_density_change", (16 + 4 + 4 + lb) * n, [&] {
            if (knz && take_warm) return go(k_compute_error<true, false, true, true>, c->stiff, PredArgs{}, NoTake{});
            if (knz) return go(k_compute_error<true, false, true>, nullptr, PredArgs{}, NoTake{});
            go(k_compute_error<true>, nullptr, PredArgs{}, NoTake{});
        });
    } else if (pred) {
        PredArgs pa = *pred;
        pa.accel = c->accel;
        pa.vel_out = c->vel2;
        launch(c, "velocity_prediction+compute_density_error", (16 + 8 + 8 + 4 + 4 + 4 + lb) * n, [&] {
            if (knz && take_warm) return go(k_compute_error<false, true, true, true>, c->kappa, pa, take_count);
            if (knz) return go(k_compute_error<false, true, true>, nullptr, pa, NoTake{});
            go(k_compute_error<false, true>, nullptr, pa, NoTake{});
        });
    } else {
        launch(c, "compute_density_error", (16 + 4 + 4 + 4 + lb) * n + (clear_hist ? 4.0 * clear_len : 0.0), [&] {
            if (knz && take_warm) return go(k_compute_error<false, false, true, true>, c->kappa, PredArgs{}, take_count);
            if (knz) return go(k_compute_error<false, false, true>, nullptr, PredArgs{}, NoTake{});
            go(k_compute_error<false>, nullptr, PredArgs{}, NoTake{});
        });
    }
}

inline bool correct_skip_ok(const sphx_ctx* c, bool divergence, float dt, const float* dt_dev, const TileClassArgs& tc, const uint32_t* knz) {
    const float inv_dt = 1.0f / dt;
    return knz && c->K.q_noclamp && !tc.pid && std::isfinite(c->K.mass) && c->K.mass > 0.0f && (dt_dev || divergence || (inv_dt > 0.0f && std::isfinite(inv_dt)));
}
void launch_correct(sphx_ctx* c, bool divergence, float dt, const float* dt_dev, const CountArgs& ca, const LoopArgs& la, const ResArgs& ra, bool first,
                    const TileClassArgs& tc, const uint32_t* knz, bool warm_taken = false) {
    const uint32_t n = c->N, f = first ? 1u : 0u;
    const float inv_dt = 1.0f / dt, lim = -0.5f * c->K.rho0 * c->K.rho0;
    const char* const label = divergence ? "correct_velocity_with_divergence_error" : "correct_velocity_with_density_error";
    float* warm = divergence ? c->stiff : c->kappa;
    const bool skip_ok = correct_skip_ok(c, divergence, dt, dt_dev, tc, knz);
    const ZeroSkipArgs zs{skip_ok ? knz : nullptr, c->zero_skip_count ? 1u : 0u};
    const bool quiet_first = zs.knz && c->quiet_hint[divergence ? 1 : 0];
    const bool thin = first && warm_taken && zs.knz && (divergence || ca.hist);
    if ((quiet_first || thin) && c->zero_skip_count) c->qf_launches += 1;
    if (thin) {
        c->thin_launches += 1;
        const uint32_t vblocks = nblocks(n);
        auto go_thin = [&](auto kernel) {
            hipLaunchKernelGGL(kernel, dim3(std::min(vblocks, c->thin_grid ? c->thin_grid : 2048u)), dim3(256), 0, c->stream, c->vel, (const float2*)c->posA,
                               (const float*)c->kbuf, warm, n, c->soff(), c->K, inv_dt, lim, c->nbv(), dt_dev, ca, c->d_scal, la, ra, zs, vblocks);
        };
        const double bytes = (16 + 8 + 12 + 8 + list_bytes(c) + (ca.hist ? 8 : 0)) * n;
        return launch(c, label, bytes, [&] { divergence ? go_thin(k_correct_thin<false>) : go_thin(k_correct_thin<true>); }, false);
    }
    auto go = [&](auto kernel, const ZeroSkipArgs& zsa) {
        hipLaunchKernelGGL(kernel, dim3(nblocks(n)), dim3(256), 0, c->stream, c->vel, (const float2*)c->posA, (const float*)c->kbuf, warm, n, c->soff(), c->K, inv_dt,
                           lim, c->nbv(), dt_dev, ca, c->d_scal, la, ra, f, tc, zsa);
    };
    launch(c, label, (16 + 8 + 12 + 8 + list_bytes(c) + (ca.hist ? (tc.pid ? 8 + 4 : 8) : 0)) * n, [&] {
        if (divergence && quiet_first) return go(k_correct<false, false, false, true, true>, zs);
        if (quiet_first) return go(k_correct<false, true, false, true, true>, zs);
        if (divergence && zs.knz) return go(k_correct<false, false, false, true>, zs);
        if (divergence) return go(k_correct<false, false>, zs);
        if (tc.pid) return go(k_correct<false, true, true>, ZeroSkipArgs{});
        if (zs.knz) return go(k_correct<false, true, false, true>, zs);
        go(k_correct<false, true>, zs);
    });
}

void launch_warmstart(sphx_ctx* c, bool divergence, float dt, const float* dt_dev, bool labelled) {
    const uint32_t n = c->N;
    const float inv_dt = 1.0f / dt, lim = -0.5f * c->K.rho0 * c->K.rho0;
    auto one = [&](auto kernel, float* warm) {
        hipLaunchKernelGGL(kernel, dim3(nblocks(n)), dim3(256), 0, c->stream, c->vel, (const float2*)c->posA, (const float*)c->kbuf, warm, n, c->soff(), c->K, inv_dt,
                           lim, c->nbv(), dt_dev, CountArgs{}, c->d_scal, LoopArgs{}, ResArgs{}, 0u, TileClassArgs{}, ZeroSkipArgs{});
    };
    auto go = [&] { divergence ? one(k_correct<true, false>, c->stiff) : one(k_correct<true, true>, c->kappa); };
    if (!labelled) return go();
    launch(c, divergence ? "correct_divergence_error_warmstart" : "correct_density_error_warmstart", (16 + 8 + 8 + 4 + list_bytes(c)) * n, go);
}

struct IterSpec {
    bool divergence, first;
    float dt;
    const float* dt_dev = nullptr;
    uint32_t* out_warm = nullptr;
    const PredArgs* pred = nullptr;
    LoopArgs la{};
    uint32_t* clear_hist = nullptr;
    uint32_t clear_len = 0;
    CountArgs ca{};
    bool drop_count = false;
    TileClassArgs tc{};
};
inline CountArgs count_args(const sphx_ctx* c, float dt) { return CountArgs{c->gdyn.view(), c->gdyn.hist, c->key, c->slot, dt}; }

uint32_t enqueue_iteration(sphx_ctx* c, const IterSpec& s) {
    if (s.out_warm && s.first) {
        const bool warm = (s.divergence ? c->num_divergence_iters : c->num_density_iters) > 1;
        *s.out_warm = warm ? 1u : 0u;
        if (warm && !(s.divergence && c->handoff.take_warm()))
            launch_warmstart(c, s.divergence, s.dt, s.dt_dev, true);
    }
    const uint32_t seq = ++c->seq;
    const ResArgs ra{1u, ++c->res_seq, c->mbox_dev, seq};
    uint32_t* knz = s.tc.pid ? nullptr : zero_skip_flags(c);
    bool warm_taken = false;
    const BuildHandoff::Taken built = c->handoff.take_first_errors(s.divergence && s.first, ra.rseq);
    if (built.fused) {
        if (!built.flags_usable) knz = nullptr;
        warm_taken = knz && built.warm_taken;
    } else {
        if (s.drop_count) drop_fused_count(c);
        warm_taken = s.first && knz && c->take_over(s.divergence) && (s.divergence || (s.ca.hist && correct_skip_ok(c, false, s.dt, s.dt_dev, s.tc, knz)));
        if (warm_taken) c->takeover_producers += 1;
        launch_compute_error(c, s.divergence, s.dt, s.dt_dev, s.la, s.clear_hist, s.clear_len, s.pred, knz, ra.rseq, warm_taken, s.ca);
    }
    if (s.pred) std::swap(c->vel, c->vel2);
    if (s.drop_count) drop_fused_count(c);
    if (s.ca.hist) s.tc.pid ? c->pending.made_by_classifier(c->N, s.dt) : c->pending.made_by_correction(c->N);
    launch_correct(c, s.divergence, s.dt, s.dt_dev, s.ca, s.la, ra, s.first, s.tc, knz, warm_taken);
    return seq;
}

uint32_t enqueue_context_iteration(sphx_ctx* c, bool divergence, float dt, const float* dt_dev, uint32_t iter, uint32_t gen, uint32_t* out_warm, bool count_ok,
                                   const PredArgs* pred = nullptr) {
    IterSpec s{divergence, iter == 1, dt, dt_dev, out_warm, pred};
    if (gen) {
        s.la.enabled = 1;
        s.la.iter = iter;
        s.la.fixed = divergence ? c->P.fixed_divergence_iterations : c->P.fixed_density_iterations;
        s.la.max_iters = divergence ? c->P.max_divergence_iterations : c->P.max_density_iterations;
        s.la.gen = gen;
        s.la.n_total = c->N;
        s.la.tol = divergence ? c->P.max_divergence_error : c->P.max_avg_density_error;
        s.la.rho0 = c->K.rho0;
        s.la.dt = dt;
    }
    if (!divergence) s.clear_len = c->gdyn.len();
    if (!divergence && count_ok && !c->no_fused_count && !c->tile_mode && c->gdyn.len()) {
        s.ca = count_args(c, dt);
        s.drop_count = !gen || s.first;
        if (!s.drop_count && c->pending.live()) s.clear_hist = c->gdyn.hist;
    }
    return enqueue_iteration(c, s);
}

int judge_residual(sphx_ctx* c, bool divergence, double err_sum, uint32_t iters, float dt, float* out_avg, bool* out_more, uint32_t* io_flags) {
    const uint32_t n = c->N;
    const float rho0 = c->K.rho0;
    const uint32_t fixed = divergence ? c->P.fixed_divergence_iterations : c->P.fixed_density_iterations;
    const uint32_t max_iters = divergence ? c->P.max_divergence_iterations : c->P.max_density_iterations;
    const float tol = divergence ? c->P.max_divergence_error : c->P.max_avg_density_error;
    const float sum = (float)err_sum;
    float avg;
    if (divergence) {
        avg = sum / (float)n / rho0;
        if (!std::isfinite(avg)) return c->fail(SPHX_ERR_NONFINITE, "avg_divergence is not finite (dfsph.rs:378)");
    } else {
        avg = sum / (float)n;
        if (!std::isfinite(avg)) return c->fail(SPHX_ERR_NONFINITE, "avg_density_error is not finite (dfsph.rs:223)");
    }
    bool more;
    if (fixed) {
        more = iters < fixed;
    } else {
        const float rel = divergence ? avg : avg / rho0;
        more = !(rel * dt < tol);
        if (more && iters > max_iters) {
            *io_flags |= divergence ? SPHX_FLAG_DIVERGENCE_ITER_CAP : SPHX_FLAG_DENSITY_ITER_CAP;
            more = false;
        }
    }
    *out_avg = avg;
    *out_more = more;
    return SPHX_OK;
}

int wait_loop(sphx_ctx* c, uint32_t seq, uint32_t gen, bool* out_done) {
    volatile uint32_t* ps = &c->mbox->seq;
    volatile uint32_t* pg = &c->mbox->loop_gen_done;
    bool done = false, reached = false;
    for (int spin = 0; spin < 400000; ++spin) {
        if (*pg == gen) {
            done = true;
            break;
        }
        if ((int32_t)(*ps - seq) >= 0) {
            reached = true;
            break;
        }
        __builtin_ia32_pause();
    }
    if (!done && !reached) {
        SPHX_HIP(c, hipStreamSynchronize(c->stream));
        done = *pg == gen;
        if (!done && (int32_t)(*ps - seq) < 0) return c->fail(SPHX_ERR_HIP, "device did not publish the solver residual (kernel fault?)");
    }
    __atomic_thread_fence(__ATOMIC_ACQUIRE);
    if (!done) done = *pg == gen;
    *out_done = done;
    return SPHX_OK;
}

uint32_t take_vmax_slot(sphx_ctx* c) {
    if (c->ahead.queued) {
        c->ahead.queued = c->ahead.valid = false;
        hipLaunchKernelGGL(k_clear_vmax_slot, dim3(1), dim3(64), 0, c->stream, c->d_scal, c->ahead.vslot);
        return c->ahead.vslot;
    }
    return c->vmax_seq++ & 3u;
}

void enqueue_nonpressure(sphx_ctx* c, float dt_prev, uint32_t vslot) {
    const uint32_t n = c->N;
    auto go = [&](auto kernel, auto visc) {
        hipLaunchKernelGGL(kernel, dim3(nblocks(n)), dim3(256), 0, c->stream, c->pv(), (const float*)c->density, n, c->soff(), c->K, dt_prev, c->nbv(), c->accel,
                           c->d_scal, vslot, visc);
    };
    launch(c, "nonpressure_accel_vmax", (16.0 + 8 + 4 + list_bytes(c)) * n, [&] {
        if (c->VK.visc_model == SPHX_VISCOSITY_PHYSICAL) return go(k_nonpressure<SPHX_VISCOSITY_PHYSICAL>, ViscArg<SPHX_VISCOSITY_PHYSICAL>{c->VK});
        go(k_nonpressure<SPHX_VISCOSITY_XSPH>, ViscArg<SPHX_VISCOSITY_XSPH>{});
    });
}

void enqueue_run_ahead(sphx_ctx* c, float dt, bool publish) {
    const uint32_t vslot = take_vmax_slot(c);
    c->ahead.queued = c->ahead.valid = true;
    c->ahead.vslot = vslot;
    c->ahead.seq = 0;
    c->ahead.n = c->N;
    std::memcpy(&c->ahead.dt_bits, &dt, 4);
    enqueue_nonpressure(c, dt, vslot);
    if (publish) {
        c->ahead.seq = ++c->seq;
        hipLaunchKernelGGL(k_publish_vmax, dim3(1), dim3(64), 0, c->stream, c->d_scal, VmaxArgs{1u, vslot, c->mbox_dev, c->ahead.seq});
    }
}

int solver_loop(sphx_ctx* c, bool divergence, float dt, uint32_t* out_iters, float* out_avg, uint32_t* out_warm, uint32_t* io_flags, bool count_ok,
                uint32_t pre_seq = 0, uint32_t pre_q = 0, uint32_t pre_gen = 0, bool run_ahead = false) {
    uint32_t iters = 0;
    float avg = 0;
    int rc;
    if (device_loop(c)) {
        const uint32_t prev = std::max(1u, divergence ? c->num_divergence_iters : c->num_density_iters);
        const uint32_t cap = (divergence ? c->P.max_divergence_iterations : c->P.max_density_iterations) + 1;
        uint32_t gen = pre_gen, q = pre_q, seq1 = pre_seq;
        if (!pre_seq) {
            if (++c->loop_gen == 0) c->loop_gen = 1;
            gen = c->loop_gen;
            seq1 = enqueue_context_iteration(c, divergence, dt, nullptr, 1, gen, out_warm, count_ok);
            q = 1;
        }
        while (q < std::min(prev, cap)) enqueue_context_iteration(c, divergence, dt, nullptr, ++q, gen, out_warm, count_ok);
        if (run_ahead && c->run_ahead) enqueue_run_ahead(c, dt, false);
        uint32_t w = q;
        for (;;) {
            bool done = false;
            if ((rc = wait_loop(c, seq1 + w - 1, gen, &done))) return rc;
            if (done) break;
            c->ahead.valid = false;
            while (q < w + 2) enqueue_context_iteration(c, divergence, dt, nullptr, ++q, gen, out_warm, count_ok);
            w += 1;
        }
        iters = c->mbox->loop_iters;
        if ((rc = wait_mailbox(c, seq1 + iters - 1))) return rc;
        c->quiet_hint[divergence ? 1 : 0] = c->mbox->quiet_seq == seq1 + iters - 1;
        const uint32_t first = iters > LOOP_HIST - 1 ? iters - (LOOP_HIST - 1) : 1;
        for (uint32_t k = first; k <= iters; ++k) {
            bool more;
            uint32_t fl = 0;
            if ((rc = judge_residual(c, divergence, c->mbox->loop_hist[k % LOOP_HIST], k, dt, &avg, &more, &fl))) return rc;
            if (more != (k < iters)) {
                c->uploaded = false;
                return c->fail(SPHX_ERR_HIP, "the device's residual test disagrees with the host's (solver loop); upload the state again");
            }
            if (k == iters) *io_flags |= fl;
        }
    } else {
        uint32_t seq = pre_seq ? pre_seq : enqueue_context_iteration(c, divergence, dt, nullptr, 1, 0, out_warm, count_ok);
        for (;;) {
            iters += 1;
            if ((rc = wait_mailbox(c, seq))) return rc;
            bool more;
            if ((rc = judge_residual(c, divergence, c->mbox->err_sum, iters, dt, &avg, &more, io_flags))) return rc;
            if (!more) {
                c->quiet_hint[divergence ? 1 : 0] = c->mbox->quiet_seq == seq;
                break;
            }
            seq = enqueue_context_iteration(c, divergence, dt, nullptr, iters + 1, 0, out_warm, count_ok);
        }
    }
    *out_iters = iters;
    *out_avg = avg;
    if (divergence)
        c->num_divergence_iters = iters;
    else
        c->num_density_iters = iters;
    return SPHX_OK;
}

}

extern "C" {

uint32_t sphx_abi_version(void) { return SPHX_ABI_VERSION; }

int sphx_default_params(float smoothing_factor, float particle_density, float fluid_density, sphx_params* p) {
    if (!p || !(particle_density > 0)) return SPHX_ERR_INVALID_ARGUMENT;
    std::memset(p, 0, sizeof(*p));
    const float radius = 0.5f / std::sqrt(particle_density);
    p->smoothing_length = 2.0f * radius * smoothing_factor;
    p->particle_mass = fluid_density / particle_density;
    p->fluid_density = fluid_density;
    p->particle_radius = radius;
    p->gravity[0] = 0.0f;
    p->gravity[1] = -9.81f;
    p->grid_min[0] = -100.0f;
    p->grid_min[1] = -100.0f;
    p->xsph_epsilon = 0.05f;
    p->viscosity_model = SPHX_VISCOSITY_XSPH;
    p->fluid_viscosity = 1.0016f / 1000.0f;
    p->max_avg_density_error = 0.01f / 100.0f;
    p->max_density_iterations = 200;
    p->max_divergence_error = 0.1f / 100.0f;
    p->max_divergence_iterations = 400;
    p->device = 0;
    return SPHX_OK;
}

const char* sphx_last_error(const sphx_ctx* ctx) { return ctx ? ctx->err.c_str() : g_create_error.c_str(); }

int sphx_debug_correction_counts(sphx_ctx* c, uint64_t out[3]) {
    if (!c || !out) return SPHX_ERR_INVALID_ARGUMENT;
    SPHX_HIP(c, hipSetDevice(c->device));
    SPHX_HIP(c, hipStreamSynchronize(c->stream));
    std::vector<Stripe> st(STRIPES);
    SPHX_HIP(c, hipMemcpy(st.data(), c->d_scal->stripe, sizeof(Stripe) * STRIPES, hipMemcpyDeviceToHost));
    out[0] = out[1] = out[2] = 0;
    for (const Stripe& s : st) {
        out[0] += s.zs_skipped;
        out[1] += s.zs_window;
        out[2] += s.zs_remote;
    }
    return SPHX_OK;
}

int sphx_debug_takeover_counts(sphx_ctx* c, uint64_t out[3]) {
    if (!c || !out) return SPHX_ERR_INVALID_ARGUMENT;
    out[0] = c->thin_launches;
    out[1] = c->takeover_producers;
    SPHX_HIP(c, hipSetDevice(c->device));
    SPHX_HIP(c, hipStreamSynchronize(c->stream));
    unsigned long long moved = 0;
    SPHX_HIP(c, hipMemcpy(&moved, &c->d_scal->spec.moved, sizeof(moved), hipMemcpyDeviceToHost));
    out[2] = moved;
    return SPHX_OK;
}

int sphx_debug_quiet_counts(sphx_ctx* c, uint64_t out[2]) {
    if (!c || !out) return SPHX_ERR_INVALID_ARGUMENT;
    SPHX_HIP(c, hipSetDevice(c->device));
    SPHX_HIP(c, hipStreamSynchronize(c->stream));
    std::vector<Stripe> st(STRIPES);
    SPHX_HIP(c, hipMemcpy(st.data(), c->d_scal->stripe, sizeof(Stripe) * STRIPES, hipMemcpyDeviceToHost));
    out[0] = 0;
    for (const Stripe& s : st) out[0] += s.zs_quiet;
    out[1] = c->qf_launches;
    return SPHX_OK;
}

int sphx_create(const sphx_params* params, sphx_ctx** out) {
    if (!params || !out) return SPHX_ERR_INVALID_ARGUMENT;
    *out = nullptr;
    if (!(params->smoothing_length > 0) || !(params->particle_mass > 0) || !(params->fluid_density > 0)) {
        g_create_error = "smoothing_length, particle_mass and fluid_density must be positive";
        return SPHX_ERR_INVALID_ARGUMENT;
    }
    if (params->viscosity_model != SPHX_VISCOSITY_XSPH && params->viscosity_model != SPHX_VISCOSITY_PHYSICAL) {
        g_create_error = "viscosity_model must be SPHX_VISCOSITY_XSPH (0) or SPHX_VISCOSITY_PHYSICAL (1)";
        return SPHX_ERR_INVALID_ARGUMENT;
    }
    if (!std::isfinite(params->fluid_viscosity)) {
        g_create_error = "fluid_viscosity must be finite";
        return SPHX_ERR_INVALID_ARGUMENT;
    }
    int ndev = 0;
    if (hipGetDeviceCount(&ndev) != hipSuccess || ndev <= 0 || params->device < 0 || params->device >= ndev) {
        g_create_error = "no usable HIP device (libsphx has no CPU fallback)";
        return SPHX_ERR_NO_DEVICE;
    }
    sphx_ctx* c = new sphx_ctx();
    if (const char* e = std::getenv("SPHX_SCAN_TWO_PASS")) c->scan_two_pass = e[0] == '1';
    if (const char* e = std::getenv("SPHX_CBITS_MIN")) c->gdyn.cbits_floor = c->gstat.cbits_floor = (uint32_t)std::max(1, std::atoi(e));
    if (const char* e = std::getenv("SPHX_NO_FUSED_COUNT")) c->no_fused_count = e[0] == '1';
    if (const char* e = std::getenv("SPHX_HOST_LOOP")) c->host_loop = e[0] == '1';
    if (const char* e = std::getenv("SPHX_RUN_AHEAD")) c->run_ahead = e[0] != '0';
    if (const char* e = std::getenv("SPHX_FUSE_PREDICT")) c->fuse_predict = e[0] != '0';
    if (const char* e = std::getenv("SPHX_LAZY_TABLE")) c->lazy_table = e[0] != '0' ? 1 : 0;
    if (const char* e = std::getenv("SPHX_STREAM_LISTS")) c->stream_lists = e[0] != '0' ? 1 : 0;
    if (const char* e = std::getenv("SPHX_NT_COLD_STORES")) c->nt_cold_stores = e[0] != '0' ? 1 : 0;
    if (const char* e = std::getenv("SPHX_TILE_FUSE_CLASS")) c->tile_fuse_class = e[0] != '0';
    if (const char* e = std::getenv("SPHX_FUSE_DIV")) c->fuse_div = e[0] != '0';
    if (const char* e = std::getenv("SPHX_XCD_CHUNK")) c->xcd_chunk = (int)xcd_shift_clamp(std::atoi(e));
    if (const char* e = std::getenv("SPHX_ALTERNATE_SWEEP")) c->alternate_sweep = e[0] == '2' ? 2 : (e[0] != '0');
    if (const char* e = std::getenv("SPHX_ZERO_SKIP")) c->zero_skip = e[0] != '0';
    if (const char* e = std::getenv("SPHX_ZERO_SKIP_COUNT")) c->zero_skip_count = e[0] == '1';
    if (const char* e = std::getenv("SPHX_QUIET_TAKEOVER")) c->quiet_takeover = std::strcmp(e, "force") == 0 ? 2 : (e[0] != '0' ? 1 : 0);
    if (const char* e = std::getenv("SPHX_QUIET_TAKEOVER_DENSITY")) c->quiet_takeover_density = e[0] != '0';
    if (const char* e = std::getenv("SPHX_THIN_GRID")) c->thin_grid = (uint32_t)std::max(0, std::atoi(e));
    if (const char* e = std::getenv("SPHX_FUSE_WARM")) c->fuse_warm = e[0] != '0';
    c->P = *params;
    c->device = params->device;
    const float h = params->smoothing_length;
    const float PI_F = (float)3.14159265358979323846;
    Consts& K = c->K;
    K.h = h;
    K.radius_sq = h * h;
    K.cell_inv = 1.0f / h;
    K.gmin_x = params->grid_min[0];
    K.gmin_y = params->grid_min[1];
    K.w_hinv = 1.0f / h;
    K.w_norm = 4.0f * 7.0f / (PI_F * rs_powi(h, 2));
    K.w_ngrad = 140.0f / (PI_F * rs_powi(h, 4));
    K.p6_hsq = h * h;
    K.p6_norm = 4.0f / (PI_F * rs_powi(h, 8));
    K.p6_ngrad = 24.0f / (PI_F * rs_powi(h, 8));
    K.sp_h = h;
    K.sp_norm = 10.0f / (PI_F * rs_powi(h, 5));
    K.sp_ngrad = 30.0f / (PI_F * rs_powi(h, 5));
    K.mass = params->particle_mass;
    K.rho0 = params->fluid_density;
    K.xsph_eps = params->xsph_epsilon;
    c->VK.visc_model = params->viscosity_model;
    c->VK.mu = params->fluid_viscosity;
    c->VK.vis_nlap = 360.0f / (29.0f * PI_F * rs_powi(h, 5));
    K.tile = TileRect{0u, 65536u, 0u, 65536u};
    K.remote_cap = params->list_span_limit == SPHX_LISTS_32BIT ? 0u : params->list_span_limit == 0 ? REMOTE_CAP : std::min(params->list_span_limit, REMOTE_CAP);
    {
        volatile float hh = h * h, root = std::sqrt(hh), qmax = h * K.w_hinv;
        c->fast_walk_ok = (root == h && qmax <= 1.0f) ? 1u : 0u;
        if (const char* e = std::getenv("SPHX_QCLAMP")) if (e[0] == '1') c->fast_walk_ok = 0u;
        K.q_noclamp = 0u;
        K.rev = 0u;
        K.nt_cold = 0u;
        K.xcd_shift = 0u;
    }
    K.gx = params->gravity[0];
    K.gy = params->gravity[1];
    {
        const float speed_of_sound = 1.0f / std::sqrt(0.01f);
        K.wc_stiffness = params->fluid_density * speed_of_sound * speed_of_sound / 7.0f;
        K.wc_boundary_force = 1.0f;
    }
    K.ax = params->gravity[0] * K.mass / K.mass;
    K.ay = params->gravity[1] * K.mass / K.mass;
    auto bail = [&](const char* what, hipError_t e) {
        g_create_error = std::string(what) + ": " + hipGetErrorString(e);
        sphx_destroy(c);
        return SPHX_ERR_HIP;
    };
    hipError_t e;
    if ((e = hipSetDevice(c->device)) != hipSuccess) return bail("hipSetDevice", e);
    if ((e = hipStreamCreateWithFlags(&c->stream, hipStreamNonBlocking)) != hipSuccess) return bail("hipStreamCreate", e);
    if ((e = hipMalloc((void**)&c->d_scal, sizeof(DevScalars))) != hipSuccess) return bail("hipMalloc", e);
    if ((e = hipHostMalloc((void**)&c->mbox, sizeof(Mailbox), hipHostMallocMapped | hipHostMallocCoherent)) != hipSuccess)
        return bail("hipHostMalloc", e);
    std::memset((void*)c->mbox, 0, sizeof(Mailbox));
    if ((e = hipHostGetDevicePointer((void**)&c->mbox_dev, (void*)c->mbox, 0)) != hipSuccess) return bail("hipHostGetDevicePointer", e);
    if ((e = hipMemsetAsync(c->d_scal, 0, sizeof(DevScalars), c->stream)) != hipSuccess) return bail("hipMemset", e);
    int rc = set_directory(c, c->gdyn, 0, 0, 0, 0, nullptr, true);
    if (!rc) rc = set_directory(c, c->gstat, 0, 0, 0, 0, nullptr, true);
    if (!rc) rc = dev_alloc(c, &c->bpos, 1);
    if (!rc) rc = dev_alloc(c, &c->bpos2, 1);
    if (!rc) rc = dev_alloc(c, &c->bid, 1);
    if (!rc) rc = dev_alloc(c, &c->bid2, 1);
    if (!rc) rc = ensure_nb_arrays(c, 0, 1, false);
    if (rc) {
        g_create_error = c->err;
        sphx_destroy(c);
        return rc;
    }
    c->capB = 1;
    *out = c;
    return SPHX_OK;
}

void sphx_destroy(sphx_ctx* c) {
    if (!c) return;
    hipSetDevice(c->device);
    if (c->stream) hipStreamSynchronize(c->stream);
#ifdef SPHX_STAMPS
// ... 16 lines not shown
    }
    for (auto e : c->ev_pool) hipEventDestroy(e);
    dev_free(&c->posA); dev_free(&c->posA2); dev_free(&c->vel); dev_free(&c->vel2); dev_free(&c->kbuf); dev_free(&c->knz); dev_free(&c->accel);
    dev_free(&c->density); dev_free(&c->alpha); dev_free(&c->alpha2); dev_free(&c->kappa); dev_free(&c->stiff); dev_free(&c->kappa2); dev_free(&c->stiff2);
    dev_free(&c->pid); dev_free(&c->pid2); dev_free(&c->key); dev_free(&c->slot); dev_free(&c->order);
    dev_free(&c->bpos); dev_free(&c->bpos2); dev_free(&c->bid); dev_free(&c->bid2); dev_free(&c->nb_list); dev_free(&c->nb_wave); dev_free(&c->nb_counts); dev_free(&c->nb_remote);
    dev_free(&c->scan_partials); dev_free(&c->scan_state); dev_free(&c->d_scal); dev_free(&c->tile_blk); dev_free(&c->sample_buf); dev_free(&c->render_buf); dev_free(&c->edit_buf); dev_free(&c->state_dig); dev_free(&c->mstate_buf);
    dev_free(&c->track.set_buf); dev_free(&c->track.rec); dev_free(&c->track.scratch); dev_free(&c->fields_buf);
    dev_free(&c->stats.scratch); dev_free(&c->stats.rec);
    free_grid(c->gdyn);
    free_grid(c->gstat);
    if (c->mbox) hipHostFree((void*)c->mbox);
    if (c->view_stream) {
        hipStreamSynchronize(c->view_stream);
        hipEventDestroy(c->view_packed);
        hipEventDestroy(c->view_done);
        hipStreamDestroy(c->view_stream);
        if (c->view_dev) hipFree(c->view_dev);
        if (c->view_host) hipHostFree(c->view_host);
    }
    if (c->stream && !c->external_stream) hipStreamDestroy(c->stream);
    delete c;
}

uint32_t sphx_num_particles(const sphx_ctx* c) { return c ? c->N : 0; }
uint32_t sphx_num_boundary(const sphx_ctx* c) { return c ? c->B : 0; }

int sphx_build_stats(const sphx_ctx* c, uint32_t* out_particles, uint64_t* out_entries, uint64_t* out_remote) {
    if (!c) return SPHX_ERR_INVALID_ARGUMENT;
    if (out_particles) *out_particles = c->N;
    if (out_entries) *out_entries = c->nb_last;
    if (out_remote) *out_remote = c->rem_last;
    return SPHX_OK;
}

int sphx_set_stream(sphx_ctx* c, void* hip_stream) {
    if (!c) return SPHX_ERR_INVALID_ARGUMENT;
    c->ahead.valid = false;
    if (c->in_step) return c->fail(SPHX_ERR_NOT_READY, "sphx_set_stream inside a step");
    SPHX_HIP(c, hipSetDevice(c->device));
    SPHX_HIP(c, hipStreamSynchronize(c->stream));
    if (c->stream && !c->external_stream) hipStreamDestroy(c->stream);
    if (hip_stream) {
        c->stream = (hipStream_t)hip_stream;
        c->external_stream = true;
    } else {
        SPHX_HIP(c, hipStreamCreateWithFlags(&c->stream, hipStreamNonBlocking));
        c->external_stream = false;
    }
    return SPHX_OK;
}

int sphx_synchronize(sphx_ctx* c) {
    if (!c) return SPHX_ERR_INVALID_ARGUMENT;
    SPHX_HIP(c, hipSetDevice(c->device));
    SPHX_HIP(c, hipStreamSynchronize(c->stream));
    return SPHX_OK;
}

int sphx_set_boundary(sphx_ctx* c, const float* xy, uint32_t n) {
    if (!c || (n && !xy)) return SPHX_ERR_INVALID_ARGUMENT;
    c->ahead.valid = false;
    if (c->in_step) return c->fail(SPHX_ERR_NOT_READY, "sphx_set_boundary between step_begin and step_finish");
    sample_went_stale(c, "sphx_set_boundary replaced the boundary (its grid is rebuilt by the next neighbour build): run a step, or "
                         "sphx_update_neighborhood + sphx_update_densities");
    SPHX_HIP(c, hipSetDevice(c->device));
    int rc;
    if (n > c->capB) {
        SPHX_HIP(c, hipStreamSynchronize(c->stream));
        if ((rc = dev_alloc(c, &c->bpos, n)) || (rc = dev_alloc(c, &c->bpos2, n)) || (rc = dev_alloc(c, &c->bid, n)) ||
            (rc = dev_alloc(c, &c->bid2, n)))
            return rc;
        if ((rc = ensure_nb_arrays(c, c->capN, n, true))) return rc;
        c->capB = n;
    }
    c->B = n;
    if (n) {
        SPHX_HIP(c, hipMemcpyAsync(c->bpos, xy, (size_t)n * 8, hipMemcpyHostToDevice, c->stream));
        hipLaunchKernelGGL(k_iota, dim3(nblocks(n)), dim3(256), 0, c->stream, c->bid, n);
        SPHX_HIP(c, hipStreamSynchronize(c->stream));
    }
    c->h_boundary.assign(xy, xy + 2 * (size_t)n);
    c->quiet_hint[0] = c->quiet_hint[1] = false;
    c->boundary_changed = true;
    return ensure_index_scratch(c);
}

int sphx_upload(sphx_ctx* c, const float* pos_xy, const float* vel_xy, uint32_t n) {
    if (!c || (n && !pos_xy)) return SPHX_ERR_INVALID_ARGUMENT;
    c->ahead.valid = false;
    if (c->in_step) return c->fail(SPHX_ERR_NOT_READY, "sphx_upload between step_begin and step_finish");
    sample_went_stale(c, "sphx_upload replaced the particles: run a step, or sphx_update_neighborhood + sphx_update_densities");
    SPHX_HIP(c, hipSetDevice(c->device));
    SPHX_HIP(c, hipStreamSynchronize(c->stream));
    clear_histograms(c);
    int rc;
    if ((rc = alloc_particles(c, n))) return rc;
    c->N = n;
    c->ids_issued = n;
    c->set_changed = false;
    lists_went_stale(c);
    if (n) {
        SPHX_HIP(c, hipMemcpyAsync(c->posA, pos_xy, (size_t)n * 8, hipMemcpyHostToDevice, c->stream));
        if (vel_xy)
            SPHX_HIP(c, hipMemcpyAsync(c->vel, vel_xy, (size_t)n * 8, hipMemcpyHostToDevice, c->stream));
        else
            SPHX_HIP(c, hipMemsetAsync(c->vel, 0, (size_t)n * 8, c->stream));
        hipLaunchKernelGGL(k_iota, dim3(nblocks(n)), dim3(256), 0, c->stream, c->pid, n);
        SPHX_HIP(c, hipStreamSynchronize(c->stream));
    }
    c->have_fluid_bbox = cell_bbox(c, pos_xy, n, c->fb);
    c->uploaded = true;
    c->gdyn.cover.clear();
    c->gdyn.nbx = c->gdyn.nby = 0;
    if (c->have_fluid_bbox && (rc = cover_dynamic(c, pos_xy, n, false))) return rc;
    return ensure_index_scratch(c);
}

int sphx_clear_cached(sphx_ctx* c) {
    if (!c) return SPHX_ERR_INVALID_ARGUMENT;
    c->ahead.valid = false;
    if (c->in_step) return c->fail(SPHX_ERR_NOT_READY, "sphx_clear_cached between step_begin and step_finish");
    SPHX_HIP(c, hipSetDevice(c->device));
    c->cached_n = 0;
    c->num_divergence_iters = 0;
    c->num_density_iters = 0;
    c->wcsph_n = 0;
    if (c->capN) {
        SPHX_HIP(c, hipMemsetAsync(c->kappa, 0, (size_t)c->capN * 4, c->stream));
        SPHX_HIP(c, hipMemsetAsync(c->stiff, 0, (size_t)c->capN * 4, c->stream));
        SPHX_HIP(c, hipMemsetAsync(c->alpha, 0, (size_t)c->capN * 4, c->stream));
    }
    return SPHX_OK;
}

int sphx_update_neighborhood(sphx_ctx* c) {
    if (!c) return SPHX_ERR_INVALID_ARGUMENT;
    c->ahead.valid = false;
    if (!c->uploaded) return c->fail(SPHX_ERR_NOT_READY, "no particles uploaded");
    if (c->in_step) return c->fail(SPHX_ERR_NOT_READY, "sphx_update_neighborhood between step_begin and step_finish");
    SPHX_HIP(c, hipSetDevice(c->device));
    int rc = update_neighborhood(c, false, 0.0f, false);
    if (rc) return rc;
    return publish_and_wait(c);
}

int sphx_update_densities(sphx_ctx* c, int kind) {
    if (!c) return SPHX_ERR_INVALID_ARGUMENT;
    c->ahead.valid = false;
    if (!c->uploaded) return c->fail(SPHX_ERR_NOT_READY, "no particles uploaded");
    SPHX_HIP(c, hipSetDevice(c->device));
    if (kind == SPHX_KERNEL_WENDLAND_C2)
        launch_density<0>(c, true, false);
    else if (kind == SPHX_KERNEL_POLY6)
        launch_density<1>(c, true, false);
    else if (kind == SPHX_KERNEL_SPIKY)
        launch_density<2>(c, true, false);
    else
        return c->fail(SPHX_ERR_INVALID_ARGUMENT, "unknown kernel kind");
    if (c->sample_ready == 1u) c->sample_ready = 2u;
    return SPHX_OK;
}

int sphx_compute_alpha(sphx_ctx* c) {
    if (!c) return SPHX_ERR_INVALID_ARGUMENT;
    c->ahead.valid = false;
// ... 4 lines not shown
}

int sphx_step_begin_law(sphx_ctx* c, float dt_prev, const sphx_timer_law* law, float* out_vmax) {
    if (!c || !out_vmax) return SPHX_ERR_INVALID_ARGUMENT;
    if (!c->uploaded) return c->fail(SPHX_ERR_NOT_READY, "sphx_step_begin before sphx_upload");
    if (c->in_step) return c->fail(SPHX_ERR_NOT_READY, "sphx_step_begin called twice");
    if (!(dt_prev > 0) || !std::isfinite(dt_prev)) return c->fail(SPHX_ERR_INVALID_ARGUMENT, "dt_prev must be positive and finite");
    if (law && (law->timestep_min_ns > law->timestep_max_ns || !(law->particle_diameter > 0) || !(law->cfl_factor > 0) || law->simulation_step_ns == 0))
        return c->fail(SPHX_ERR_INVALID_ARGUMENT, "sphx_timer_law: need 0 < min <= max, a positive diameter, cfl factor and current step");
    SPHX_HIP(c, hipSetDevice(c->device));
    sample_went_stale(c, "the last DFSPH step did not finish: run a step, or sphx_update_neighborhood + sphx_update_densities");
    const bool ahead_ok = c->ahead.queued && c->ahead.valid;
    c->ahead.valid = false;
    c->step_flags = 0;
    c->step_dt_prev = dt_prev;
    c->pre_seq = 0;
    c->law_active = false;
    const uint32_t n = c->N;
    int rc;
    if (c->cached_n != n || c->set_changed) {
        c->set_changed = false;
        if (n > c->cached_n) {
            const uint32_t add = n - c->cached_n;
            for (float* a : {c->alpha, c->kappa, c->stiff})
                hipLaunchKernelGGL(k_fill_f32, dim3(nblocks(add)), dim3(256), 0, c->stream, a, c->cached_n, n, 0.0f);
        }
        c->cached_n = n;
        if ((rc = update_neighborhood(c, true, 0.0f, true))) return rc;
        c->step_flags |= SPHX_FLAG_WARMUP;
    }
    if (n == 0) {
        *out_vmax = 0.0f;
        c->step_vmax = 0.0f;
        c->in_step = true;
        return SPHX_OK;
    }
    TimerLaw tl{};
    if (law) {
        tl.enabled = 1;
        tl.adaptive = law->adaptive ? 1u : 0u;
        tl.cfl_factor = law->cfl_factor;
        tl.particle_diameter = law->particle_diameter;
        tl.min_ns = law->timestep_min_ns;
        tl.max_ns = law->timestep_max_ns;
        tl.step_ns = law->simulation_step_ns;
    }
    const uint32_t seq = ++c->seq;
    uint32_t dt_prev_bits;
    std::memcpy(&dt_prev_bits, &dt_prev, 4);
    const bool adopted = ahead_ok && !(c->step_flags & SPHX_FLAG_WARMUP) && c->ahead.n == n && c->ahead.dt_bits == dt_prev_bits;
    uint32_t vslot;
    if (adopted) {
        vslot = c->ahead.vslot;
        c->ahead.queued = false;
    } else {
        vslot = take_vmax_slot(c);
        enqueue_nonpressure(c, dt_prev, vslot);
    }
    const VmaxArgs va{1u, vslot, c->mbox_dev, seq};
    if (!law) hipLaunchKernelGGL(k_publish_vmax, dim3(1), dim3(64), 0, c->stream, c->d_scal, va);
    if (law) {
        const float* dt_dev = &c->d_scal->dt;
        const bool fuse_pred = c->fuse_predict && c->num_density_iters <= 1;
        PredArgs pa{};
        pa.va = va;
        pa.law = tl;
        const PredArgs* const pred = fuse_pred ? &pa : nullptr;
        if (!fuse_pred)
            launch_predict(c, "velocity_prediction", 1.0f, va, tl);
        if (device_loop(c)) {
            if (++c->loop_gen == 0) c->loop_gen = 1;
            c->pre_gen = c->loop_gen;
            const uint32_t want = std::min(std::max(1u, c->num_density_iters), c->P.max_density_iterations + 1);
            c->pre_seq = enqueue_context_iteration(c, false, 1.0f, dt_dev, 1, c->pre_gen, &c->pre_warm, true, pred);
            for (c->pre_queued = 1; c->pre_queued < want;) enqueue_context_iteration(c, false, 1.0f, dt_dev, ++c->pre_queued, c->pre_gen, &c->pre_warm, true);
        } else {
            c->pre_gen = 0;
            c->pre_queued = 1;
            c->pre_seq = enqueue_context_iteration(c, false, 1.0f, dt_dev, 1, 0, &c->pre_warm, true, pred);
        }
        c->law_active = true;
    }
    if ((rc = wait_mailbox(c, seq))) return rc;
    const uint32_t vbits = c->mbox->vmax_sq_bits;
    float vsq;
    std::memcpy(&vsq, &vbits, 4);
    if (!std::isfinite(vsq)) return c->fail(SPHX_ERR_NONFINITE, "max velocity is not finite (Duration::from_secs_f32 would panic, timemanager.rs:264)");
    c->step_vmax = std::sqrt(vsq);
    c->law_dt_bits = c->mbox->dt_bits;
    *out_vmax = c->step_vmax;
    c->in_step = true;
    return SPHX_OK;
}

int sphx_step_begin(sphx_ctx* c, float dt_prev, float* out_vmax) { return sphx_step_begin_law(c, dt_prev, nullptr, out_vmax); }

int sphx_step_finish(sphx_ctx* c, float dt, sphx_step_stats* out) {
    if (!c) return SPHX_ERR_INVALID_ARGUMENT;
    if (!c->in_step || c->in_wcsph) return c->fail(SPHX_ERR_NOT_READY, "sphx_step_finish without sphx_step_begin");
    c->in_step = false;
    if (!(dt > 0) || !std::isfinite(dt)) {
        if (c->law_active) c->uploaded = false;
        c->law_active = false;
        drop_fused_count(c);
        return c->fail(SPHX_ERR_INVALID_ARGUMENT, c->uploaded ? "dt must be positive and finite"
                                                               : "dt must be positive and finite (phase B had started: upload the state again)");
    }
    SPHX_HIP(c, hipSetDevice(c->device));
    const uint32_t n = c->N;
    sphx_step_stats s;
    std::memset(&s, 0, sizeof(s));
    s.dt_prev = c->step_dt_prev;
    s.dt = dt;
    s.vmax = c->step_vmax;
    int rc;
    auto broken = [&](int code) {
        if (code == SPHX_ERR_HIP || code == SPHX_ERR_NONFINITE) {
            c->uploaded = false;
            clear_histograms(c);
        }
        drop_fused_count(c);
        c->ahead.valid = false;
        c->handoff.clear();
        c->law_active = false;
        return code;
    };
    if (n) {
        uint32_t pre = 0, pre_q = 0, pre_gen = 0;
        if (c->law_active) {
            uint32_t bits;
            std::memcpy(&bits, &dt, 4);
            if (bits != c->law_dt_bits) {
                c->uploaded = false;
                c->law_active = false;
                drop_fused_count(c);
                return c->fail(SPHX_ERR_INVALID_ARGUMENT, "dt differs from the sphx_timer_law handed to sphx_step_begin_law; upload the state again");
            }
            pre = c->pre_seq;
            pre_q = c->pre_queued;
            pre_gen = c->pre_gen;
            s.warmstart_density = c->pre_warm;
        } else {
            launch_predict(c, "velocity_prediction", dt);
        }
        c->law_active = false;
        if ((rc = solver_loop(c, false, dt, &s.density_iterations, &s.avg_density_error, &s.warmstart_density, &c->step_flags, true, pre, pre_q, pre_gen)))
            return broken(rc);
        const bool fuse_div = c->fuse_div && !c->tile_mode && c->num_divergence_iters <= 1;
        const bool fuse_warm = c->fuse_div && c->fuse_warm && !c->tile_mode && c->num_divergence_iters > 1;
        if ((rc = update_neighborhood(c, false, dt, true, fuse_div, fuse_warm))) return broken(rc);
        if ((rc = solver_loop(c, true, dt, &s.divergence_iterations, &s.avg_divergence, &s.warmstart_divergence, &c->step_flags, false, 0, 0, 0, true)))
            return broken(rc);
        s.neighbor_entries = c->nb_last;
        s.remote_entries = (uint32_t)std::min<unsigned long long>(c->rem_last, 0xFFFFFFFFull);
    }
    c->law_active = false;
    s.flags = c->step_flags;
    if (out) *out = s;
    sample_after_step(c);
    track_after_step(c);
    stats_after_step(c, dt);
    return SPHX_OK;
}

int sphx_wcsph_step_begin(sphx_ctx* c, float dt, float* out_vmax) {
    if (!c || !out_vmax) return SPHX_ERR_INVALID_ARGUMENT;
    c->ahead.valid = false;
    if (!c->uploaded) return c->fail(SPHX_ERR_NOT_READY, "sphx_wcsph_step_begin before sphx_upload");
    if (c->in_step) return c->fail(SPHX_ERR_NOT_READY, "a step is already open");
    if (c->tile_mode) return c->fail(SPHX_ERR_INVALID_ARGUMENT, "WCSPH is not available on tiles");
    if (!(dt > 0) || !std::isfinite(dt)) return c->fail(SPHX_ERR_INVALID_ARGUMENT, "dt must be positive and finite");
    SPHX_HIP(c, hipSetDevice(c->device));
    sample_went_stale(c, "the last WCSPH step did not finish: run a step, or sphx_update_neighborhood + sphx_update_densities");
    c->step_flags = 0;
    c->step_dt_prev = dt;
    const uint32_t n = c->N;
    *out_vmax = 0.0f;
    c->step_vmax = 0.0f;
    if (n == 0) {
        c->in_step = true;
        c->in_wcsph = true;
        return SPHX_OK;
    }
    hipStream_t st = c->stream;
    const dim3 g(nblocks(n)), b(256);
    if (c->wcsph_n < n)
        SPHX_HIP(c, hipMemsetAsync(c->accel + c->wcsph_n, 0, (size_t)(n - c->wcsph_n) * 8, st));
    c->wcsph_n = n;
    launch(c, "wcsph_leapfrog1", 40.0 * n, [&] { hipLaunchKernelGGL(k_wcsph_leapfrog1, g, b, 0, st, c->vel, c->posA, (const float2*)c->accel, n, dt); });
    int rc;
    if ((rc = update_neighborhood(c, false, 0.0f, false))) return rc;
    launch_density<1>(c, true, false);
    const uint32_t seq = ++c->seq;
    const VmaxArgs va{1u, take_vmax_slot(c), c->mbox_dev, seq};
    launch(c, "wcsph_accelerations_vmax", (16.0 + 4 + 8 + 4 + list_bytes(c)) * n, [&] {
        if (c->VK.visc_model == SPHX_VISCOSITY_PHYSICAL)
            hipLaunchKernelGGL(k_wcsph_accel<SPHX_VISCOSITY_PHYSICAL>, g, b, 0, st, c->pv(), (const float*)c->density, n, c->soff(), c->K, dt, c->nbv(),
                               c->accel, c->d_scal, va.vslot, ViscArg<SPHX_VISCOSITY_PHYSICAL>{c->VK});
        else
            hipLaunchKernelGGL(k_wcsph_accel<SPHX_VISCOSITY_XSPH>, g, b, 0, st, c->pv(), (const float*)c->density, n, c->soff(), c->K, dt, c->nbv(),
                               c->accel, c->d_scal, va.vslot, ViscArg<SPHX_VISCOSITY_XSPH>{});
    });
    hipLaunchKernelGGL(k_publish_vmax, dim3(1), dim3(64), 0, st, c->d_scal, va);
    if ((rc = wait_mailbox(c, seq))) return rc;
    const uint32_t vbits = c->mbox->vmax_sq_bits;
    float vsq;
// ... 668 lines not shown
```

Before: 12.75 billion.

## Skip nonpressure neighbour walk when all velocities are identical (rigid motion)

Adds a 'rigid' fast path. The gather kernel marks whether any particle velocity differs from particle 0's. When the previous step proved every velocity uniform, the nonpressure kernel writes gravity-only acceleration instead of walking neighbours, because viscosity terms vanish for uniform velocity. The kernel still checks device-side marks and falls back to the full walk in a grid-stride loop when velocities differ. It only turns on for N >= 4M without tiling. It adds bookkeeping, a judge kernel, a ballot in the gather, and host-side hint state.

```diff
diff --git a/include/sphx.h b/include/sphx.h
--- a/include/sphx.h
+++ b/include/sphx.h
@@ -197,6 +197,9 @@
 int sphx_debug_correction_counts(sphx_ctx* ctx, uint64_t out[3]);
 int sphx_debug_quiet_counts(sphx_ctx* ctx, uint64_t out[2]);
 int sphx_debug_takeover_counts(sphx_ctx* ctx, uint64_t out[3]);
+
+int sphx_debug_rigid_counts(sphx_ctx* ctx, uint64_t out[3]);
+int sphx_debug_download_accel(sphx_ctx* ctx, float* out_xy);
 
 int sphx_clear_cached(sphx_ctx* ctx);
 int sphx_step_begin(sphx_ctx* ctx, float dt_prev, float* out_vmax);
diff --git a/yasph2d_amd/__init__.py b/yasph2d_amd/__init__.py
--- a/yasph2d_amd/__init__.py
+++ b/yasph2d_amd/__init__.py
@@ -546,6 +546,16 @@
         self._chk(self.L.sphx_debug_takeover_counts(self.h, out))
         return int(out[0]), int(out[1]), int(out[2])
 
+    def rigid_counts(self):
+        out = (C.c_uint64 * 3)()
+        self._chk(self.L.sphx_debug_rigid_counts(self.h, out))
+        return int(out[0]), int(out[1]), int(out[2])
+
+    def download_accel(self):
+        out = np.zeros((self.n, 2), np.float32)
+        self._chk(self.L.sphx_debug_download_accel(self.h, out.ctypes.data_as(C.c_void_p)))
+        return out
+
     def grid_info(self, which=0):
         out = (C.c_uint32 * 4)()
         self._chk(self.L.sphx_grid_info(self.h, which, out))
diff --git a/yasph2d_amd/_lib.py b/yasph2d_amd/_lib.py
--- a/yasph2d_amd/_lib.py
+++ b/yasph2d_amd/_lib.py
@@ -243,6 +243,8 @@
     "sphx_debug_correction_counts": (_i, [_vp, _vp]),
     "sphx_debug_quiet_counts": (_i, [_vp, _vp]),
     "sphx_debug_takeover_counts": (_i, [_vp, _vp]),
+    "sphx_debug_rigid_counts": (_i, [_vp, _vp]),
+    "sphx_debug_download_accel": (_i, [_vp, _vp]),
     "sphx_download_by_id": (_i, [_vp, _u32, _u32, _u32, C.POINTER(SphxTrackOut), C.POINTER(_u32)]),
     "sphx_download": (_i, [_vp, _vp, _vp, _vp, _vp]),
     "sphx_download_boundary": (_i, [_vp, _vp, _vp]),
diff --git a/yasph2d_amd/csrc/sphx_handoff.hpp b/yasph2d_amd/csrc/sphx_handoff.hpp
--- a/yasph2d_amd/csrc/sphx_handoff.hpp
+++ b/yasph2d_amd/csrc/sphx_handoff.hpp
@@ -68,4 +68,26 @@
     uint32_t n_ = 0, dt_bits_ = 0;
 };
 
+struct VelMarks {
+    bool valid = false, thin_seen = false;
+    uint32_t tag = 0, knz_tag = 0;
+    struct Taken {
+        bool usable, check_knz;
+        uint32_t tag, knz_tag;
+    };
+    void made(uint32_t gather_tag) { *this = VelMarks{true, false, gather_tag, 0u}; }
+    void thin(uint32_t rseq) {
+        if (!valid) return;
+        if (thin_seen) return wrote();
+        thin_seen = true;
+        knz_tag = rseq;
+    }
+    void wrote() { *this = VelMarks{}; }
+    Taken take() {
+        const Taken t{valid, valid && thin_seen, tag, knz_tag};
+        wrote();
+        return t;
+    }
+};
+
 }
diff --git a/yasph2d_amd/csrc/sphx_internal.hpp b/yasph2d_amd/csrc/sphx_internal.hpp
--- a/yasph2d_amd/csrc/sphx_internal.hpp
+++ b/yasph2d_amd/csrc/sphx_internal.hpp
@@ -133,8 +133,10 @@
 };
 struct alignas(128) MarkStripe {
     uint32_t knz_mark;
-    uint32_t pad[31];
-};
+    uint32_t vmix_mark;
+    uint32_t pad[30];
+};
+static_assert(sizeof(MarkStripe) == 128, "one stripe, one cache line");
 struct alignas(128) SpecLine {
     uint32_t flags;
     uint32_t pad0;
@@ -149,7 +151,8 @@
     uint32_t loop_done;
     uint32_t pad0;
     unsigned long long snap_hi[2], snap_lo[2];
-    uint32_t pad[18];
+    uint32_t rigid_exits, rigid_marked;
+    uint32_t pad[16];
     Stripe stripe[STRIPES];
     VmaxStripe vstripe[STRIPES];
     MarkStripe mstripe[STRIPES];
@@ -172,6 +175,7 @@
     uint32_t loop_iters;
     double loop_hist[LOOP_HIST];
     uint32_t send_counts[MAX_TILE_PEERS];
+    uint32_t rigid_tag;
 };
 
 struct ResArgs {
@@ -308,6 +312,18 @@
         return !tile_mode && (divergence || quiet_takeover_density) && (quiet_takeover == 2 || (quiet_takeover == 1 && quiet_hint[divergence ? 1 : 0]));
     }
     unsigned long long thin_launches = 0, takeover_producers = 0;
+    int rigid_skip = -1;
+    bool rigid_on() const { return !tile_mode && (rigid_skip < 0 ? N >= 4000000u : rigid_skip != 0); }
+    sphx::VelMarks velmarks;
+    uint32_t gather_seq = 0;
+    bool rigid_hint = false;
+    uint32_t rigid_judged = 0;
+    void rigid_forget() {
+        velmarks.wrote();
+        rigid_hint = false;
+        rigid_judged = 0;
+    }
+    unsigned long long rigid_launches = 0;
     float2* accel = nullptr;
     float *density = nullptr, *alpha = nullptr, *alpha2 = nullptr, *kappa = nullptr, *stiff = nullptr;
     float *kappa2 = nullptr, *stiff2 = nullptr;
@@ -409,6 +425,7 @@
 
     int fail(int code, const char* what, const char* detail = nullptr) {
         quiet_hint[0] = quiet_hint[1] = false;
+        rigid_forget();
         err = what;
         if (detail) {
             err += ": ";
diff --git a/yasph2d_amd/csrc/sphx_kernels.hip b/yasph2d_amd/csrc/sphx_kernels.hip
--- a/yasph2d_amd/csrc/sphx_kernels.hip
+++ b/yasph2d_amd/csrc/sphx_kernels.hip
@@ -664,6 +664,7 @@
     TileRect own;
     uint32_t rank_by_id;
     uint32_t nt_cold;
+    uint32_t vmix_tag;
 };
 #ifndef SPHX_GATHER_PER_LANE
 #define SPHX_GATHER_PER_LANE 1
@@ -675,6 +676,9 @@
     if (n_dev) n = min(n, *n_dev);
     const uint32_t b0 = xcd_bid(xcd_packed_rev(rev), xcd_packed_shift(rev)) * (256u * GATHER_PER_LANE);
     if (b0 >= n) return;
+    uint2 vref = make_uint2(0u, 0u);
+    if (a.vmix_tag) vref = *(const uint2*)a.vel_in;
+    bool vmix = false;
     constexpr int RANK_L = 5, RANK_R = 6;
     constexpr uint32_t ORD_HALO = 8, SPAN = 256u * GATHER_PER_LANE;
     static_assert(RANK_L <= (int)ORD_HALO && RANK_R <= (int)ORD_HALO, "window of order[] words in LDS");
@@ -766,6 +770,7 @@
                 qd.y = qd.y + v[u].y * a.advect_dt;
             }
             a.vel_out[dst] = v[u];
+            vmix = vmix || __float_as_uint(v[u].x) != vref.x || __float_as_uint(v[u].y) != vref.y;
         }
         a.pos_out[dst] = qd;
         if (a.r_in) a.r_out[dst] = r1[u];
@@ -784,6 +789,11 @@
                     atomicAdd(&a.count_owned->stripe[blockIdx.x % STRIPES].owned, (unsigned long long)__popcll(m));
             }
         }
+    }
+    if (a.vmix_tag) {
+        const bool ref_bad = (vref.x & 0x7f800000u) == 0x7f800000u || (vref.y & 0x7f800000u) == 0x7f800000u;
+        const unsigned long long m = __ballot(vmix || ref_bad);
+        if (m && (threadIdx.x & 63) == (uint32_t)(__ffsll((long long)__ballot(1)) - 1)) a.flags->mstripe[blockIdx.x % STRIPES].vmix_mark = a.vmix_tag;
     }
 }
 
@@ -2075,70 +2085,69 @@
                                                       ViscArg<VM> V) {
     __shared__ Stage<2, 1> rec;
     const uint32_t blk = xcd_bid(K.rev, K.xcd_shift);
-    const uint32_t i = blk * 256 + threadIdx.x;
-    NbHead h = nb_head(nb, blk, i, n);
-    struct StageRec {
-        float4 pv;
-        float rho;
-    };
-    nb_stage(
-        h, nb, blk, i, n, [&](uint32_t g) { return StageRec{ldpv(PV, g), gat(density, g < soff ? g : 0u)}; },
-        [&](uint32_t g) {
-            const Pair<float4> pv = ldpv2(PV, g);
-            const Pair<float> rho = gat2(density, g < soff ? g : 0u);
-            return Pair<StageRec>{StageRec{pv.a, rho.a}, StageRec{pv.b, rho.b}};
-        },
-        [&](uint32_t slot, const StageRec& r) {
-            rec.put_vec01(slot, r.pv);
-            rec.put_scal<0>(slot, r.rho);
-        });
+#include "sphx_nonpressure_body.inc"
+    block_vmax_add(vsq, scal, vslot, (uint32_t*)&rec.raw[0]);
+}
+
+struct RigidArgs {
+    uint32_t vmix_tag;
+    uint32_t knz_tag;
+    uint32_t check_knz;
+    uint32_t vgrid;
+    Mailbox* mb;
+};
+__device__ __forceinline__ bool rigid_marked(const DevScalars* __restrict__ scal, float rho0, float dt, const RigidArgs& ra) {
+    uint32_t vm = ~ra.vmix_tag, km = ~ra.knz_tag;
+    if ((threadIdx.x & 63u) < STRIPES) {
+        vm = scal->mstripe[threadIdx.x & 63u].vmix_mark;
+        km = scal->mstripe[threadIdx.x & 63u].knz_mark;
+    }
+    const float rd = rho0 * dt;
+    const bool dt_ok = dt > 0.0f && dt <= 3.402823466e38f && rd >= 1.175494351e-38f && rd <= 3.402823466e38f;
+    return __any(vm == ra.vmix_tag || (ra.check_knz != 0u && km == ra.knz_tag)) != 0 || !dt_ok;
+}
+template <int VM>
+__global__ NONP_BOUNDS void k_nonpressure_rigid(PVr PV, const float* __restrict__ density, uint32_t n, uint32_t soff, Consts K,
+                                                            float dt, NbView nb, float2* __restrict__ accel, DevScalars* __restrict__ scal, uint32_t vslot,
+                                                            ViscArg<VM> V, RigidArgs ra) {
+    __shared__ Stage<2, 1> rec;
+    uint32_t* const wm = (uint32_t*)&rec.raw[0];
+    if (threadIdx.x < 64) {
+        const bool m = rigid_marked(scal, K.rho0, dt, ra);
+        if (threadIdx.x == 0) wm[0] = m ? 1u : 0u;
+    }
     __syncthreads();
-    float vsq = 0.0f;
-    if (i < n) {
-        const uint32_t oi = (i - h.lw0) * 4u;
-        const float4 pvi = h.wide ? ldpv(PV, i) : rec.vec01(oi);
-        const uint32_t cd = h.cd;
-        float ax = K.ax, ay = K.ay;
-        struct Rec {
-            float4 pv;
-            float rho;
-        };
-        if constexpr (VM == SPHX_VISCOSITY_PHYSICAL) {
-            const float mu_m = V.mu * K.mass;
-            auto walk = [&](auto fast) {
-                auto consume = [&](const Rec& r, uint32_t) {
-                    const float dx = r.pv.x - pvi.x, dy = r.pv.y - pvi.y;
-                    const float r_sq = dx * dx + dy * dy;
-                    const float f = physical_visc(K, V, mu_m, sqrt_dist<decltype(fast)::value>(r_sq), r.rho);
-                    ax = ax + f * (r.pv.z - pvi.z);
-                    ay = ay + f * (r.pv.w - pvi.w);
-                };
-                nb_traverse(
-                    h, cd, [&](uint32_t o) { return Rec{rec.vec01(o), rec.scal<0>(o)}; },
-                    [&](uint32_t g) { return Rec{ldpv(PV, g), gat(density, g)}; }, consume);
-            };
-            if (K.q_noclamp)
-                walk(std::true_type{});
-            else
-                walk(std::false_type{});
-        } else {
-            const float em = K.xsph_eps * K.mass;
-            auto consume = [&](const Rec& r, uint32_t) {
-                const float dx = r.pv.x - pvi.x, dy = r.pv.y - pvi.y;
-                const float r_sq = dx * dx + dy * dy;
-                const float f = em * poly6_eval(K, r_sq) / (r.rho * dt);
-                ax = ax + f * (r.pv.z - pvi.z);
-                ay = ay + f * (r.pv.w - pvi.w);
-            };
-            nb_traverse(
-                h, cd, [&](uint32_t o) { return Rec{rec.vec01(o), rec.scal<0>(o)}; },
-                [&](uint32_t g) { return Rec{ldpv(PV, g), gat(density, g)}; }, consume);
-        }
-        accel[i] = make_float2(ax, ay);
-        const float px = pvi.z + ax * dt, py = pvi.w + ay * dt;
-        vsq = tile_owns(K, pvi.x, pvi.y) ? px * px + py * py : 0.0f;
-    }
-    block_vmax_add(vsq, scal, vslot, (uint32_t*)&rec.raw[0]);
+    const bool marked = wm[0] != 0u;
+    if (blockIdx.x == 0 && threadIdx.x == 0) {
+        __hip_atomic_store(&ra.mb->rigid_tag, marked ? 0u : ra.vmix_tag, __ATOMIC_RELAXED, __HIP_MEMORY_SCOPE_SYSTEM);
+        atomicAdd(marked ? &scal->rigid_marked : &scal->rigid_exits, 1u);
+    }
+    if (!marked) {
+        const float2 a = make_float2(K.ax, K.ay);
+        for (uint32_t vblk = blockIdx.x; vblk < ra.vgrid; vblk += gridDim.x) {
+            const uint32_t i = xcd_map(vblk, ra.vgrid, K.rev, K.xcd_shift) * 256u + threadIdx.x;
+            if (i < n) accel[i] = a;
+        }
+        if (blockIdx.x == 0 && threadIdx.x == 0) {
+            const float2 v = PV.vel[0];
+            const float px = v.x + a.x * dt, py = v.y + a.y * dt;
+            const uint32_t m = __float_as_uint(px * px + py * py);
+            if (m) atomicMax(&scal->vstripe[0].vmax[vslot & 3u], m);
+        }
+        return;
+    }
+    uint32_t vbits = 0u;
+    for (uint32_t vblk = blockIdx.x; vblk < ra.vgrid; vblk += gridDim.x) {
+        __syncthreads();
+        const uint32_t blk = xcd_map(vblk, ra.vgrid, K.rev, K.xcd_shift);
+#include "sphx_nonpressure_body.inc"
+        vbits = max(vbits, __float_as_uint(vsq));
+    }
+    block_vmax_add(__uint_as_float(vbits), scal, vslot, wm);
+}
+__global__ __launch_bounds__(64) void k_rigid_judge(const DevScalars* __restrict__ scal, float rho0, float dt, RigidArgs ra) {
+    const bool marked = rigid_marked(scal, rho0, dt, ra);
+    if (threadIdx.x == 0) __hip_atomic_store(&ra.mb->rigid_tag, marked ? 0u : ra.vmix_tag, __ATOMIC_RELAXED, __HIP_MEMORY_SCOPE_SYSTEM);
 }
 
 __global__ __launch_bounds__(256) void k_predict(float2* __restrict__ vel, const float2* __restrict__ accel, uint32_t n, float dt,
diff --git a/yasph2d_amd/csrc/sphx_launch.inc b/yasph2d_amd/csrc/sphx_launch.inc
--- a/yasph2d_amd/csrc/sphx_launch.inc
+++ b/yasph2d_amd/csrc/sphx_launch.inc
@@ -519,7 +519,8 @@
     flush_pending_advect(c);
 }
 
-int build_grid(sphx_ctx* c, Grid& g, const float2* pos, uint32_t n, const GatherArgs& ga, float advect_dt, bool ring, uint32_t* tile_n = nullptr) {
+int build_grid(sphx_ctx* c, Grid& g, const float2* pos, uint32_t n, const GatherArgs& ga, float advect_dt, bool ring, uint32_t* tile_n = nullptr,
+               bool mark_velocities = false) {
     hipStream_t st = c->stream;
     DevScalars* ds = c->d_scal;
     const uint32_t len = g.len();
@@ -527,6 +528,7 @@
     const bool counted = &g == &c->gdyn && advect_dt > 0 && !tile_n && c->pending.is_for(n);
     const bool partial = &g == &c->gdyn && tile_n && advect_dt == 0.0f && !counted && c->pending.is_for_first_of(n);
     const uint32_t first = partial ? c->pending.n() : 0u;
+    if (&g == &c->gdyn) c->velmarks.wrote();
     if (counted || partial)
         c->pending.forget();
     else
@@ -582,11 +584,17 @@
         if (ga.r2_in) gbytes += 8;
         if (ga.r3_in) gbytes += 8;
         if (ga.u_in) gbytes += 8;
+        GatherArgs gm = ga;
+        if (mark_velocities && &g == &c->gdyn && !tile_n && ga.vel_in) {
+            if (++c->gather_seq == 0) c->gather_seq = 1;
+            gm.vmix_tag = c->gather_seq;
+        }
         if (ng)
             launch(c, "gather_attributes", gbytes * ng, [&] {
                 hipLaunchKernelGGL(k_rank_gather, dim3(gb2), dim3(256), 0, st, (const uint32_t*)c->order, (const uint32_t*)c->key, ng, n,
-                                   (const uint2*)g.fine, ga, tile_n ? (const uint32_t*)&ds->sort_total : (const uint32_t*)nullptr, g.cbits(), xcd_pack(c->K.rev, xcd_shift_of(c)));
+                                   (const uint2*)g.fine, gm, tile_n ? (const uint32_t*)&ds->sort_total : (const uint32_t*)nullptr, g.cbits(), xcd_pack(c->K.rev, xcd_shift_of(c)));
             });
+        if (ng && gm.vmix_tag) c->velmarks.made(gm.vmix_tag);
     }
     return SPHX_OK;
 }
@@ -629,6 +637,7 @@
     c->K.q_noclamp = 0u;
     c->lists_current = false;
     c->quiet_hint[0] = c->quiet_hint[1] = false;
+    c->rigid_forget();
     if (c->d_scal) hipMemsetAsync(&c->d_scal->spec.flags, 0, sizeof(uint32_t), c->stream);
     if (c->sample_ready) sample_went_stale(c, "the positions changed since the last neighbour build: run a step, or sphx_update_neighborhood + sphx_update_densities");
 }
@@ -807,7 +816,9 @@
             flush_pending_advect(c);
         }
     }
-    if ((rc = build_grid(c, c->gdyn, c->posA, c->N, ga, advect_dt, true, c->tile_mode ? &tile_n : nullptr))) return rc;
+    const bool take_div = fuse && fuse_div && !fuse_warm && zero_skip_flags(c) && c->take_over(true);
+    if ((rc = build_grid(c, c->gdyn, c->posA, c->N, ga, advect_dt, true, c->tile_mode ? &tile_n : nullptr, take_div && advect_dt > 0.0f && c->rigid_on())))
+        return rc;
     if (carry_kappa) std::swap(c->kappa, c->kappa2);
     if (carry_stiff) std::swap(c->stiff, c->stiff2);
     std::swap(c->vel, c->vel2);
@@ -831,13 +842,14 @@
             dv.lim = -0.5f * c->K.rho0 * c->K.rho0;
             launch(c, "neighbor_build+density_alpha+divergence_warmstart", (8.0 + list_bytes(c) + 8.0 + 8.0 + 8.0 + 4.0) * n, [&] { go(k_neighbor_build<3>, dv); });
             c->handoff = BuildHandoff::warm_applied();
+            c->velmarks.wrote();
         } else if (fuse && fuse_div) {
             DivArgs dv{};
             dv.vel = (const float2*)c->vel;
             dv.kbuf = c->kbuf;
             dv.knz = zero_skip_flags(c);
             dv.knz_tag = c->res_seq + 1u;
-            const bool take = dv.knz && c->take_over(true);
+            const bool take = take_div;
             if (take) {
                 dv.warm = c->stiff;
                 c->takeover_producers += 1;
@@ -932,6 +944,7 @@
 
 void launch_predict(sphx_ctx* c, const char* label, float dt, const VmaxArgs& va = VmaxArgs{}, const TimerLaw& tl = TimerLaw{}) {
     const uint32_t n = c->N;
+    c->velmarks.wrote();
     launch(c, label, 24.0 * n, [&] { hipLaunchKernelGGL(k_predict, dim3(nblocks(n)), dim3(256), 0, c->stream, c->vel, (const float2*)c->accel, n, dt, c->d_scal, va, tl); });
 }
 
@@ -940,6 +953,7 @@
                           const CountArgs& take_count = CountArgs{}) {
     const uint32_t n = c->N;
     const double lb = list_bytes(c);
+    if (pred) c->velmarks.wrote();
     auto go = [&](auto kernel, float* warm, const PredArgs& pa, auto take) {
         hipLaunchKernelGGL(kernel, dim3(nblocks(n)), dim3(256), 0, c->stream, c->pv(), (const float*)c->density, (const float*)c->alpha, n, c->soff(), c->K, dt,
                            c->nbv(), c->kbuf, warm, c->d_scal, dt_dev, la, clear_hist, clear_len, pa, knz, knz_tag, take);
@@ -983,6 +997,7 @@
     const bool quiet_first = zs.knz && c->quiet_hint[divergence ? 1 : 0];
     const bool thin = first && warm_taken && zs.knz && (divergence || ca.hist);
     if ((quiet_first || thin) && c->zero_skip_count) c->qf_launches += 1;
+    thin ? c->velmarks.thin(ra.rseq) : c->velmarks.wrote();
     if (thin) {
         c->thin_launches += 1;
         const uint32_t vblocks = nblocks(n);
@@ -1010,6 +1025,7 @@
 
 void launch_warmstart(sphx_ctx* c, bool divergence, float dt, const float* dt_dev, bool labelled) {
     const uint32_t n = c->N;
+    c->velmarks.wrote();
     const float inv_dt = 1.0f / dt, lim = -0.5f * c->K.rho0 * c->K.rho0;
     auto one = [&](auto kernel, float* warm) {
         hipLaunchKernelGGL(kernel, dim3(nblocks(n)), dim3(256), 0, c->stream, c->vel, (const float2*)c->posA, (const float*)c->kbuf, warm, n, c->soff(), c->K, inv_dt,
@@ -1152,11 +1168,38 @@
     return c->vmax_seq++ & 3u;
 }
 
-void enqueue_nonpressure(sphx_ctx* c, float dt_prev, uint32_t vslot) {
+inline bool finite_not_neg_zero(float f) {
+    uint32_t u;
+    std::memcpy(&u, &f, 4);
+    return std::isfinite(f) && u != 0x80000000u;
+}
+inline bool rigid_conditions(const sphx_ctx* c, float dt) {
+    const float rd = c->K.rho0 * dt;
+    const float fc = c->VK.visc_model == SPHX_VISCOSITY_PHYSICAL ? c->VK.mu * c->K.mass * c->VK.vis_nlap * c->K.h : c->K.xsph_eps * c->K.mass * c->K.p6_norm;
+    return c->rigid_on() && c->K.q_noclamp && c->lists_current && finite_not_neg_zero(c->K.ax) && finite_not_neg_zero(c->K.ay) && dt > 0.0f &&
+           std::isfinite(dt) && std::isfinite(rd) && rd >= 1.175494351e-38f && std::isfinite(fc);
+}
+void enqueue_nonpressure(sphx_ctx* c, float dt_prev, uint32_t vslot, const VelMarks::Taken& marks = VelMarks::Taken{}) {
     const uint32_t n = c->N;
+    const bool judged = marks.usable && rigid_conditions(c, dt_prev);
+    const RigidArgs ra{marks.tag, marks.knz_tag, marks.check_knz ? 1u : 0u, nblocks(n), c->mbox_dev};
+    c->rigid_judged = judged ? marks.tag : 0u;
+    if (!judged) c->rigid_hint = false;
+    if (judged && (c->rigid_skip == 2 || c->rigid_hint)) {
+        c->rigid_launches += 1;
+        auto go_rigid = [&](auto kernel, auto visc) {
+            hipLaunchKernelGGL(kernel, dim3(std::min(ra.vgrid, c->thin_grid ? c->thin_grid : 2048u)), dim3(256), 0, c->stream, c->pv(), (const float*)c->density, n,
+                               c->soff(), c->K, dt_prev, c->nbv(), c->accel, c->d_scal, vslot, visc, ra);
+        };
+        return launch(c, "nonpressure_accel_vmax", 8.0 * n, [&] {
+            if (c->VK.visc_model == SPHX_VISCOSITY_PHYSICAL) return go_rigid(k_nonpressure_rigid<SPHX_VISCOSITY_PHYSICAL>, ViscArg<SPHX_VISCOSITY_PHYSICAL>{c->VK});
+            go_rigid(k_nonpressure_rigid<SPHX_VISCOSITY_XSPH>, ViscArg<SPHX_VISCOSITY_XSPH>{});
+        }, false);
+    }
     auto go = [&](auto kernel, auto visc) {
         hipLaunchKernelGGL(kernel, dim3(nblocks(n)), dim3(256), 0, c->stream, c->pv(), (const float*)c->density, n, c->soff(), c->K, dt_prev, c->nbv(), c->accel,
                            c->d_scal, vslot, visc);
+        if (judged) hipLaunchKernelGGL(k_rigid_judge, dim3(1), dim3(64), 0, c->stream, (const DevScalars*)c->d_scal, c->K.rho0, dt_prev, ra);
     };
     launch(c, "nonpressure_accel_vmax", (16.0 + 8 + 4 + list_bytes(c)) * n, [&] {
         if (c->VK.visc_model == SPHX_VISCOSITY_PHYSICAL) return go(k_nonpressure<SPHX_VISCOSITY_PHYSICAL>, ViscArg<SPHX_VISCOSITY_PHYSICAL>{c->VK});
@@ -1171,7 +1214,7 @@
     c->ahead.seq = 0;
     c->ahead.n = c->N;
     std::memcpy(&c->ahead.dt_bits, &dt, 4);
-    enqueue_nonpressure(c, dt, vslot);
+    enqueue_nonpressure(c, dt, vslot, publish ? VelMarks::Taken{} : c->velmarks.take());
     if (publish) {
         c->ahead.seq = ++c->seq;
         hipLaunchKernelGGL(k_publish_vmax, dim3(1), dim3(64), 0, c->stream, c->d_scal, VmaxArgs{1u, vslot, c->mbox_dev, c->ahead.seq});
@@ -1299,6 +1342,26 @@
     return SPHX_OK;
 }
 
+int sphx_debug_rigid_counts(sphx_ctx* c, uint64_t out[3]) {
+    if (!c || !out) return SPHX_ERR_INVALID_ARGUMENT;
+    out[0] = c->rigid_launches;
+    SPHX_HIP(c, hipSetDevice(c->device));
+    SPHX_HIP(c, hipStreamSynchronize(c->stream));
+    uint32_t dev[2] = {0u, 0u};
+    SPHX_HIP(c, hipMemcpy(dev, &c->d_scal->rigid_exits, sizeof(dev), hipMemcpyDeviceToHost));
+    out[1] = dev[0];
+    out[2] = dev[1];
+    return SPHX_OK;
+}
+
+int sphx_debug_download_accel(sphx_ctx* c, float* out_xy) {
+    if (!c || (c->N && !out_xy)) return SPHX_ERR_INVALID_ARGUMENT;
+    SPHX_HIP(c, hipSetDevice(c->device));
+    SPHX_HIP(c, hipStreamSynchronize(c->stream));
+    if (c->N) SPHX_HIP(c, hipMemcpy(out_xy, c->accel, (size_t)c->N * 8, hipMemcpyDeviceToHost));
+    return SPHX_OK;
+}
+
 int sphx_debug_quiet_counts(sphx_ctx* c, uint64_t out[2]) {
     if (!c || !out) return SPHX_ERR_INVALID_ARGUMENT;
     SPHX_HIP(c, hipSetDevice(c->device));
@@ -1349,6 +1412,7 @@
     if (const char* e = std::getenv("SPHX_ZERO_SKIP_COUNT")) c->zero_skip_count = e[0] == '1';
     if (const char* e = std::getenv("SPHX_QUIET_TAKEOVER")) c->quiet_takeover = std::strcmp(e, "force") == 0 ? 2 : (e[0] != '0' ? 1 : 0);
     if (const char* e = std::getenv("SPHX_QUIET_TAKEOVER_DENSITY")) c->quiet_takeover_density = e[0] != '0';
+    if (const char* e = std::getenv("SPHX_RIGID_SKIP")) c->rigid_skip = std::strcmp(e, "force") == 0 ? 2 : (e[0] != '0' ? 1 : 0);
     if (const char* e = std::getenv("SPHX_THIN_GRID")) c->thin_grid = (uint32_t)std::max(0, std::atoi(e));
     if (const char* e = std::getenv("SPHX_FUSE_WARM")) c->fuse_warm = e[0] != '0';
     c->P = *params;
@@ -1531,6 +1595,7 @@
     }
     c->h_boundary.assign(xy, xy + 2 * (size_t)n);
     c->quiet_hint[0] = c->quiet_hint[1] = false;
+    c->rigid_forget();
     c->boundary_changed = true;
     return ensure_index_scratch(c);
 }
@@ -1701,6 +1766,10 @@
         c->law_active = true;
     }
     if ((rc = wait_mailbox(c, seq))) return rc;
+    if (c->rigid_judged) {
+        c->rigid_hint = c->mbox->rigid_tag == c->rigid_judged;
+        c->rigid_judged = 0;
+    }
     const uint32_t vbits = c->mbox->vmax_sq_bits;
     float vsq;
     std::memcpy(&vsq, &vbits, 4);
@@ -1741,6 +1810,7 @@
         drop_fused_count(c);
         c->ahead.valid = false;
         c->handoff.clear();
+        c->rigid_forget();
         c->law_active = false;
         return code;
     };
diff --git a/yasph2d_amd/csrc/sphx_nonpressure_body.inc b/yasph2d_amd/csrc/sphx_nonpressure_body.inc
--- /dev/null
+++ b/yasph2d_amd/csrc/sphx_nonpressure_body.inc
@@ -0,0 +1,63 @@
+    const uint32_t i = blk * 256 + threadIdx.x;
+    NbHead h = nb_head(nb, blk, i, n);
+    struct StageRec {
+        float4 pv;
+        float rho;
+    };
+    nb_stage(
+        h, nb, blk, i, n, [&](uint32_t g) { return StageRec{ldpv(PV, g), gat(density, g < soff ? g : 0u)}; },
+        [&](uint32_t g) {
+            const Pair<float4> pv = ldpv2(PV, g);
+            const Pair<float> rho = gat2(density, g < soff ? g : 0u);
+            return Pair<StageRec>{StageRec{pv.a, rho.a}, StageRec{pv.b, rho.b}};
+        },
+        [&](uint32_t slot, const StageRec& r) {
+            rec.put_vec01(slot, r.pv);
+            rec.put_scal<0>(slot, r.rho);
+        });
+    __syncthreads();
+    float vsq = 0.0f;
+    if (i < n) {
+        const uint32_t oi = (i - h.lw0) * 4u;
+        const float4 pvi = h.wide ? ldpv(PV, i) : rec.vec01(oi);
+        const uint32_t cd = h.cd;
+        float ax = K.ax, ay = K.ay;
+        struct Rec {
+            float4 pv;
+            float rho;
+        };
+        if constexpr (VM == SPHX_VISCOSITY_PHYSICAL) {
+            const float mu_m = V.mu * K.mass;
+            auto walk = [&](auto fast) {
+                auto consume = [&](const Rec& r, uint32_t) {
+                    const float dx = r.pv.x - pvi.x, dy = r.pv.y - pvi.y;
+                    const float r_sq = dx * dx + dy * dy;
+                    const float f = physical_visc(K, V, mu_m, sqrt_dist<decltype(fast)::value>(r_sq), r.rho);
+                    ax = ax + f * (r.pv.z - pvi.z);
+                    ay = ay + f * (r.pv.w - pvi.w);
+                };
+                nb_traverse(
+                    h, cd, [&](uint32_t o) { return Rec{rec.vec01(o), rec.scal<0>(o)}; },
+                    [&](uint32_t g) { return Rec{ldpv(PV, g), gat(density, g)}; }, consume);
+            };
+            if (K.q_noclamp)
+                walk(std::true_type{});
+            else
+                walk(std::false_type{});
+        } else {
+            const float em = K.xsph_eps * K.mass;
+            auto consume = [&](const Rec& r, uint32_t) {
+                const float dx = r.pv.x - pvi.x, dy = r.pv.y - pvi.y;
+                const float r_sq = dx * dx + dy * dy;
+                const float f = em * poly6_eval(K, r_sq) / (r.rho * dt);
+                ax = ax + f * (r.pv.z - pvi.z);
+                ay = ay + f * (r.pv.w - pvi.w);
+            };
+            nb_traverse(
+                h, cd, [&](uint32_t o) { return Rec{rec.vec01(o), rec.scal<0>(o)}; },
+                [&](uint32_t g) { return Rec{ldpv(PV, g), gat(density, g)}; }, consume);
+        }
+        accel[i] = make_float2(ax, ay);
+        const float px = pvi.z + ax * dt, py = pvi.w + ay * dt;
+        vsq = tile_owns(K, pvi.x, pvi.y) ? px * px + py * py : 0.0f;
+    }
```

Measured after the change: 13.43 billion (median of 6 runs). 5.3% higher.
